# engcang/FAST-LIO-SAM-QN

Measured on AMD Instinct MI355X. Metric: scan-pair registrations/sec on 100k-pt clouds, higher is better.
Workload: dtype f32 search / f64 accumulate

## Files before the change

### fast-lio-sam-qn_amd/csrc/qn_context.h

```cpp
#pragma once
#include <hip/hip_runtime.h>
#include <string>
#include <vector>
#include "qn_gicp_kernels.cuh"

struct CloudBuf {
  uint32_t n = 0, ncells = 0;
  bool has_grid = false, has_cov = false;
  float4* raw = nullptr;
  float4* sorted = nullptr;
  float4* sorted_tmp = nullptr;
  uint32_t* cell_of_pt = nullptr;
  uint32_t* cell_start = nullptr;
  uint32_t* counts = nullptr;
  double* nrm = nullptr;
  qn::GridView grid{};
  qn::GridDims* dims = nullptr;
  qn::GridDims* dims_host = nullptr;
  const int32_t* knn_tab = nullptr; int knn_k = 0;
};

struct ProfSpan { int family; hipEvent_t a, b; int count; };

struct qn_ctx {
  int device = 0;
  uint32_t max_points = 0, max_cells = 0;
  hipStream_t stream = nullptr; bool owns_stream = true;
  std::vector<qn_ctx*> lanes; int batch_lanes = 8; char* args_h = nullptr; char* args_d = nullptr; size_t args_cap = 0; uint64_t batch_launches = 0, batch_pairs = 0; bool is_lane = false, batch_trace = false, batch_share_source = true;
  bool lanes_failed = false; int fail_lane_create = 0;
  void* slab = nullptr;
  qn_gicp_params params{};
  CloudBuf cloud[2];
  qn::BBoxAcc* bbox_acc = nullptr; qn::BBoxAcc* bbox_acc2 = nullptr;
  unsigned long long* scan_status = nullptr; unsigned long long* scan_status2 = nullptr; uint32_t build_epoch = 0;
  int far_group = -1;
  int far_chunk = 2;
  bool batch_look = false;
  bool far_ranked = true;
  unsigned long long* list_probe = nullptr;
  bool device_look = true;
  bool clear_far_now = false;
  char* staging2 = nullptr;
  struct PinZone { char* h = nullptr; hipEvent_t ev = nullptr; bool busy = false; } pin_up, pin_up2;
  char* staging = nullptr;
  uint32_t* scan_sums = nullptr;

  qn::GicpState* state = nullptr;
  uint32_t gen = 0; int part_rows = 0;
  double* partials = nullptr;
  uint32_t* tail_ticket = nullptr;
  double* fit_psum = nullptr; uint32_t* fit_pcnt = nullptr;
  qn_iter_trace* trace = nullptr; uint32_t trace_len = 0;
  int32_t* corr = nullptr; int32_t* nn_idx = nullptr; int32_t* knn_idx = nullptr; float4* nn_ref = nullptr; double* nrm_s_sorted = nullptr; qn::TargetRec* tgt_rec = nullptr; float* sqd = nullptr; float* sqd_fit = nullptr;
  int32_t* far_cand = nullptr; float4* far_cand_ref = nullptr; float2* far_cand_b = nullptr; unsigned long long* far_req = nullptr; uint32_t* far_stats = nullptr; double* far_rows = nullptr; int far_mode = 2; bool far_enabled = true;
  uint2* fb_list = nullptr; uint2* big_list = nullptr; uint32_t* fb_count2 = nullptr;
  float4* aligned = nullptr; bool aligned_valid = false;
  double* pose_tmp = nullptr; float* guess_tmp = nullptr;
  qn::ResultBlock* result_host = nullptr; double* scalar_host = nullptr;
  int32_t* dbg_knn_idx = nullptr; float* dbg_knn_d2 = nullptr;
  qn_quatro_params qparams{}; bool qparams_set = false, q_ready = false; double q_last_scale = 1.0;
  float4* q_normals[2] = {nullptr, nullptr}; float* q_spfh[2] = {nullptr, nullptr}; float* q_fpfh_s[2] = {nullptr, nullptr}; float* q_fpfh[2] = {nullptr, nullptr};
  unsigned long long* q_key[2] = {nullptr, nullptr};
  float* q_pair[2] = {nullptr, nullptr}; uint32_t* q_pair_hash[2] = {nullptr, nullptr};
  uint32_t* q_hit = nullptr; uint32_t* q_list = nullptr; uint32_t* q_sel = nullptr; uint2* q_pairs = nullptr; uint32_t* q_counts = nullptr; double* q_T = nullptr;
  void* q_mm_c = nullptr; void* q_mm_q = nullptr; float* q_mm_qn = nullptr; uint32_t* q_mm_L = nullptr; unsigned long long* q_mm_table = nullptr; unsigned long long* q_mm_table_q = nullptr; bool feat_query_dedupe = false;
  uint32_t q_mm_mask = 0;
  uint2* q_mm_pairs = nullptr; uint32_t* q_mm_cnt = nullptr; uint32_t q_mm_cap = 0, q_mm_ncnt = 0; bool feat_mfma = true, feat_mm_retry = false; int feat_sample = 4 ; bool feat_verify = false; int feat_min_blocks = 1536; double q_wall_ms[3] = {0, 0, 0}; unsigned long long* q_mm_vkeys = nullptr; uint32_t* q_mm_vcnt = nullptr; uint32_t feat_fallbacks = 0, feat_survivors = 0;
  bool c2f_overlap = false;
  bool c2f_lanes_fpfh = false;
  bool tgt_early = true;
  bool quatro_fused = true;
  int normals_fg = 0, fpfh_fg = 0;
  float4* c2f_src = nullptr; float4* c2f_dst = nullptr;
  float* q_mean = nullptr; double* q_mean_psum = nullptr; void* q_host = nullptr;
  double cell_override = 0.0;
  int list_small = 6000;
  float big_ratio = 2.5f;
  bool fused_ticks = true;
  int nn_rounds = 1;
  int nn_lane = -1;
  int track_from_tick = 3;
  int fused_from_tick = 3;
  int unseeded_until = 3; bool count_far_now = false; int last_extra_unseeded = 0;
  int unseeded_cap = 10;
  int single_from_tick = 2;
  bool fused_final = true;
  int knn_rounds = 2;
  int knn_mm = 1;
  int knn_trips = 3;
  int knn_hist = 1;
  int big_blocks0 = 4096, fb_blocks0 = 512;
  float margin_nn_t0 = 0.f;
  float margin_nn = 1.f, margin_knn = 0.f;
  int margin_nn_cap = 3, margin_knn_cap = 5, ticks_per_chunk = 8; bool knn_single_all = false, stable_cells = true; int bbox_blocks = 64;
  hipStream_t stream2 = nullptr; hipEvent_t ev_pair = nullptr; bool pair_pipeline = true, pair_failed = false, tgt_on_stream2 = false, tgt_pending = false, no_pipe = false;
// ... 24 lines not shown
```

### fast-lio-sam-qn_amd/csrc/qn_device.cuh

```cuda
#pragma once
#include <hip/hip_runtime.h>
#include <stdint.h>

namespace qn {

#define QN_TX 8
#define QN_TY 4
#define QN_TZ 4
#define QN_TILE_CELLS 128

struct GridDims {
  float ox, oy, oz, cell, inv_cell, eps;
  int nx, ny, nz, ntx, nty, ntz;
  uint32_t n;
  uint32_t ncells, nonfinite, pad;
};
struct GridView {
  const float4* pts;
  const uint32_t* cell_start;
  uint32_t* dbg;
  float ox, oy, oz, cell, inv_cell, eps;
  int nx, ny, nz;
  int ntx, nty, ntz;
  uint32_t n;
  const GridDims* dims;
};
__device__ __forceinline__ int uni(int v) { return __builtin_amdgcn_readfirstlane(v); }
__device__ __forceinline__ uint32_t uni(uint32_t v) { return (uint32_t)__builtin_amdgcn_readfirstlane((int)v); }
__device__ __forceinline__ float uni(float v) { return __int_as_float(__builtin_amdgcn_readfirstlane(__float_as_int(v))); }
__device__ __forceinline__ double uni(double v) { union { double d; int i[2]; } u; u.d = v; u.i[0] = __builtin_amdgcn_readfirstlane(u.i[0]); u.i[1] = __builtin_amdgcn_readfirstlane(u.i[1]); return u.d; }
__device__ __forceinline__ GridView grid_resolve(GridView g) {
  const GridDims d = *g.dims;
  g.ox = uni(d.ox); g.oy = uni(d.oy); g.oz = uni(d.oz); g.cell = uni(d.cell); g.inv_cell = uni(d.inv_cell); g.eps = uni(d.eps);
  g.nx = uni(d.nx); g.ny = uni(d.ny); g.nz = uni(d.nz); g.ntx = uni(d.ntx); g.nty = uni(d.nty); g.ntz = uni(d.ntz); g.n = uni(d.n);
  return g;
}

template <class A> struct alignas(16) LaneEntry { A a; uint32_t nbx; uint32_t pad_[3]; };
template <class F>
__global__ void __launch_bounds__(F::TB, F::OCC) k_lanes(const LaneEntry<typename F::Args>* __restrict__ tab) {
  const LaneEntry<typename F::Args>* e = tab + blockIdx.y;
  const uint32_t nbx = e->nbx;
  if (blockIdx.x >= nbx) return;
  F::run(e->a, blockIdx.x, nbx);
}

#define QN_INF_KEY 0xFFFFFFFFFFFFFFFFull

__device__ __forceinline__ int clampi(int v, int lo, int hi) { return v < lo ? lo : (v > hi ? hi : v); }
__device__ __forceinline__ int cell_coord(float v, float o, float inv, int n) {
  return clampi((int)floorf((v - o) * inv), 0, n - 1);
}
__device__ __forceinline__ uint32_t cell_key(const GridView& g, int x, int y, int z) {
  const uint32_t tile = ((uint32_t)(z >> 2) * g.nty + (y >> 2)) * g.ntx + (x >> 3);
  return (tile << 7) | ((z & 3) << 5) | ((y & 3) << 3) | (x & 7);
}
__device__ __forceinline__ unsigned long long pack_key(float d2, uint32_t idx) {
  return ((unsigned long long)__float_as_uint(d2) << 32) | idx;
}
__device__ __forceinline__ float key_d2(unsigned long long k) { return __uint_as_float((uint32_t)(k >> 32)); }
__device__ __forceinline__ uint32_t key_idx(unsigned long long k) { return (uint32_t)k; }

typedef float qn_f2 __attribute__((ext_vector_type(2)));
__device__ __forceinline__ float sqdist(float qx, float qy, float qz, float px, float py, float pz) {
  const qn_f2 q = {qx, qy}, p = {px, py};
  const qn_f2 d = q - p;
  const qn_f2 d2 = d * d;
  const float dz = qz - pz;
  return (d2.x + d2.y) + dz * dz;
}

__device__ __forceinline__ int rfl(int v) { return __builtin_amdgcn_readfirstlane(v); }
__device__ __forceinline__ uint32_t rflu(uint32_t v) { return (uint32_t)__builtin_amdgcn_readfirstlane((int)v); }
__device__ __forceinline__ int rdlane(int v, int l) { return __builtin_amdgcn_readlane(v, l); }
__device__ __forceinline__ uint32_t rdlane(uint32_t v, int l) { return (uint32_t)__builtin_amdgcn_readlane((int)v, l); }
__device__ __forceinline__ float rdlane(float v, int l) { return __int_as_float(__builtin_amdgcn_readlane(__float_as_int(v), l)); }

#if defined(QN_INST_GROUP) && QN_INST_GROUP == 10
__device__ __forceinline__ int wave_min_i(int v) {
#pragma unroll
  for (int o = 32; o > 0; o >>= 1) { int t = __shfl_xor(v, o); v = t < v ? t : v; }
  return v;
}
__device__ __forceinline__ int wave_max_i(int v) {
#pragma unroll
  for (int o = 32; o > 0; o >>= 1) { int t = __shfl_xor(v, o); v = t > v ? t : v; }
  return v;
}
__device__ __forceinline__ unsigned long long wave_min_u64(unsigned long long v) {
#pragma unroll
  for (int o = 32; o > 0; o >>= 1) { unsigned long long t = __shfl_xor(v, o); v = t < v ? t : v; }
  return v;
}
__device__ __forceinline__ float wave_min_f(float v) {
#pragma unroll
  for (int o = 32; o > 0; o >>= 1) v = fminf(v, __shfl_xor(v, o));
  return v;
}
__device__ __forceinline__ float wave_max_f(float v) {
#pragma unroll
  for (int o = 32; o > 0; o >>= 1) v = fmaxf(v, __shfl_xor(v, o));
  return v;
}
#else
#define QN_DPP_LADDER(STEP) STEP(0x111, 0xF) STEP(0x112, 0xF) STEP(0x114, 0xF) STEP(0x118, 0xF) STEP(0x142, 0xA) STEP(0x143, 0xC)
__device__ __forceinline__ int wave_min_i(int v) {
#define QN_S(ctrl, rm) { const int t = __builtin_amdgcn_update_dpp(0x7fffffff, v, ctrl, rm, 0xF, false); v = t < v ? t : v; }
  QN_DPP_LADDER(QN_S)
// ... 777 lines not shown
```

### fast-lio-sam-qn_amd/csrc/qn_engine.hip

```cpp
#include <hip/hip_runtime.h>
#include <cfloat>
#include <cmath>
#include <cstdio>
#include <cstring>
#include <string>
#include <vector>
#include <atomic>
#include <thread>
#include <chrono>
#include "qn_instances.h"
#include "qn_context.h"
#include "qn_selftest.cuh"
#include "qn_pool.h"

using namespace qn;

#define HIPCHK(ctx, call)                                                                 \
  do { hipError_t e_ = (call);                                                            \
       if (e_ != hipSuccess) { (ctx)->set_error(#call, e_, __LINE__); return QN_ERR_HIP; } \
  } while (0)

void qn_ctx::set_error(const char* what, hipError_t e, int line) {
  char buf[512]; snprintf(buf, sizeof(buf), "%s -> %s (qn_engine.hip:%d)", what, hipGetErrorString(e), line);
  last_error = buf;
}

void qn_ctx::prof_begin(int family, int count) {
  if (!prof_on) return;
  if (prof_open) { prof_depth++; return; }
  ProfSpan sp; sp.family = family; sp.count = count;
  if (hipEventCreate(&sp.a) != hipSuccess) return;
  if (hipEventCreate(&sp.b) != hipSuccess) { hipEventDestroy(sp.a); return; }
  hipEventRecord(sp.a, stream);
  spans.push_back(sp);
  prof_open = true; prof_depth = 0;
}
void qn_ctx::prof_end() {
  if (!prof_on || spans.empty() || !prof_open) return;
  if (prof_depth > 0) { prof_depth--; return; }
  prof_open = false;
  hipEventRecord(spans.back().b, stream);
}
void qn_ctx::prof_collect() {
  for (auto& sp : spans) {
    float ms = 0; if (hipEventSynchronize(sp.b) == hipSuccess && hipEventElapsedTime(&ms, sp.a, sp.b) == hipSuccess) { stats[sp.family].total_ms += ms; stats[sp.family].launches += sp.count; }
    hipEventDestroy(sp.a); hipEventDestroy(sp.b);
  }
  spans.clear(); prof_open = false; prof_depth = 0;
}
struct ProfScope { qn_ctx* c; ProfScope(qn_ctx* c_, int fam) : c(c_) { c->prof_begin(fam); } ~ProfScope() { c->prof_end(); } };

extern "C" const char* qn_status_str(int s) {
  switch (s) {
    case QN_OK: return "ok"; case QN_ERR_INVALID_ARG: return "invalid argument"; case QN_ERR_EMPTY_CLOUD: return "empty cloud";
    case QN_ERR_CAPACITY: return "cloud exceeds context capacity"; case QN_ERR_NOT_READY: return "clouds/covariances not set";
    case QN_ERR_HIP: return "HIP runtime error"; case QN_ERR_NO_DEVICE: return "no gfx950 device (no CPU fallback)";
  }
  return "unknown status";
}
extern "C" const char* qn_last_error(const qn_ctx* ctx) { return ctx ? ctx->last_error.c_str() : "null context"; }

extern "C" void qn_gicp_default_params(qn_gicp_params* p) {
  if (!p) return;
  memset(p, 0, sizeof(*p));
  p->k_correspondences = 20; p->max_iterations = 64; p->max_corr_dist = (double)FLT_MAX;
  p->transformation_epsilon = 5e-4; p->rotation_epsilon = 2e-3; p->optimizer = QN_OPT_LM;
  p->lm_max_iterations = 10; p->lm_init_lambda_factor = 1e-9; p->force_iterations = 0;
  p->ransac_iterations = 0; p->ransac_outlier_threshold = 0.05; p->euclidean_fitness_epsilon = -DBL_MAX;
}

struct Slab {
  char* base = nullptr; size_t off = 0, cap = 0;
  template <class T> void take(T*& p, size_t bytes) {
    const size_t a = (off + 255) & ~(size_t)255;
    if (base) p = (T*)(base + a);
    off = a + bytes;
  }
};
static void carve_cloud(qn_ctx* c, Slab& sl, CloudBuf& b) {
  sl.take(b.raw, sizeof(float4) * c->max_points);
  sl.take(b.sorted, sizeof(float4) * c->max_points);
  sl.take(b.sorted_tmp, sizeof(float4) * c->max_points);
  sl.take(b.cell_of_pt, sizeof(uint32_t) * c->max_points);
  sl.take(b.cell_start, sizeof(uint32_t) * ((size_t)c->max_cells + 1));
  sl.take(b.counts, sizeof(uint32_t) * ((size_t)c->max_cells + 1));
  sl.take(b.nrm, sizeof(double) * 3 * c->max_points);
  sl.take(b.dims, sizeof(GridDims));
}

static int ctx_create(int device, uint32_t max_points, hipStream_t shared_stream, qn_ctx** out);
extern "C" int qn_ctx_create(int device, uint32_t max_points, qn_ctx** out) { return ctx_create(device, max_points, nullptr, out); }
static int ctx_create(int device, uint32_t max_points, hipStream_t shared_stream, qn_ctx** out) {
  if (!out || max_points == 0) return QN_ERR_INVALID_ARG;
  *out = nullptr;
  if (max_points > QN_CTX_MAX_POINTS) return QN_ERR_CAPACITY;
  int ndev = 0;
  if (hipGetDeviceCount(&ndev) != hipSuccess || ndev <= 0 || device < 0 || device >= ndev) return QN_ERR_NO_DEVICE;
  qn_ctx* c = new qn_ctx();
  c->device = device; c->max_points = max_points;
  size_t mc = (size_t)max_points * 16; if (mc < (1u << 18)) mc = 1u << 18; if (mc > (1u << 23)) mc = 1u << 23;
  c->max_cells = (uint32_t)mc;
  qn_gicp_default_params(&c->params);
  int rc = QN_OK;
  auto fail = [&](int code) { qn_ctx_destroy(c); return code; };
  if (hipSetDevice(device) != hipSuccess) return fail(QN_ERR_NO_DEVICE);
  if (shared_stream) { c->stream = shared_stream; c->owns_stream = false; c->is_lane = true; }
  else if (hipStreamCreateWithFlags(&c->stream, hipStreamNonBlocking) != hipSuccess) return fail(QN_ERR_HIP);
#define CA(call) if ((call) != hipSuccess) return fail(QN_ERR_HIP)
  auto carve = [&](Slab& sl) {
    carve_cloud(c, sl, c->cloud[0]);
    carve_cloud(c, sl, c->cloud[1]);
    sl.take(c->staging, (size_t)max_points * 32);
    sl.take(c->scan_sums, sizeof(uint32_t) * (c->max_cells / (QN_BLOCK * QN_SCAN_ITEMS) + 2));
    sl.take(c->state, 2 * sizeof(GicpState));
    sl.take(c->partials, 2 * sizeof(double) * (QN_ACC_MAX_BLOCKS + 8) * QN_NPART);
    sl.take(c->nn_idx, sizeof(int32_t) * max_points);
    sl.take(c->knn_idx, sizeof(int32_t) * (size_t)max_points * 32);
    sl.take(c->nn_ref, sizeof(float4) * max_points);
    sl.take(c->nrm_s_sorted, sizeof(double) * 3 * max_points);
    sl.take(c->tgt_rec, sizeof(TargetRec) * max_points);
    sl.take(c->fit_psum, sizeof(double) * (QN_ACC_MAX_BLOCKS + 8));
    sl.take(c->fit_pcnt, sizeof(uint32_t) * (QN_ACC_MAX_BLOCKS + 8));
    sl.take(c->trace, sizeof(qn_iter_trace) * QN_MAX_TRACE);
    sl.take(c->corr, sizeof(int32_t) * max_points);
    sl.take(c->sqd, sizeof(float) * max_points);
    sl.take(c->sqd_fit, sizeof(float) * max_points);
    sl.take(c->far_cand, sizeof(int32_t) * QN_FAR_M * (size_t)max_points);
    sl.take(c->far_cand_ref, sizeof(float4) * max_points);
    sl.take(c->far_cand_b, sizeof(float2) * max_points);
    sl.take(c->far_req, sizeof(unsigned long long) * (max_points / 64 + 2));
    sl.take(c->far_stats, 4 * sizeof(uint32_t));
    sl.take(c->far_rows, sizeof(double) * QN_FAR_BLOCKS * QN_NPART);
    sl.take(c->fb_list, sizeof(uint2) * max_points);
    sl.take(c->big_list, sizeof(uint2) * max_points);
    sl.take(c->fb_count2, 4 * sizeof(uint32_t));
    sl.take(c->aligned, sizeof(float4) * max_points);
    sl.take(c->pose_tmp, sizeof(double) * 16);
    sl.take(c->guess_tmp, sizeof(float) * 16);
    sl.take(c->scan_sums2, sizeof(uint32_t) * (c->max_cells / (QN_BLOCK * QN_SCAN_ITEMS) + 2));
    sl.take(c->fb_list2, sizeof(uint2) * max_points);
    sl.take(c->big_list2, sizeof(uint2) * max_points);
    sl.take(c->fb_count2b, 4 * sizeof(uint32_t));
    sl.take(c->knn_idx2, sizeof(int32_t) * (size_t)max_points * 32);
    sl.take(c->staging2, (size_t)max_points * 32);
    sl.take(c->bbox_acc, 2 * (QN_BBOX_MAX_BLOCKS + 1) * sizeof(BBoxAcc)); c->bbox_acc2 = c->bbox_acc ? c->bbox_acc + (QN_BBOX_MAX_BLOCKS + 1) : nullptr;
    sl.take(c->scan_status, sizeof(unsigned long long) * 2 * (c->max_cells / (QN_BLOCK * QN_SCAN_ITEMS) + 2)); c->scan_status2 = c->scan_status ? c->scan_status + (c->max_cells / (QN_BLOCK * QN_SCAN_ITEMS) + 2) : nullptr;
    sl.take(c->pg_rows, sizeof(unsigned long long) * 3 * QN_PERSIST_ROWS * QN_PERSIST_RSTRIDE);
    sl.take(c->pg_bc, sizeof(unsigned long long) * 64);
    sl.take(c->pg_fit, sizeof(unsigned long long) * (QN_PERSIST_MAX_BLOCKS + 1) * 4);
    sl.take(c->pg_status, 4 * sizeof(uint32_t));
    sl.take(c->tail_ticket, 4 * sizeof(uint32_t));
  };
  { Slab dry; carve(dry);
    Slab sl; sl.cap = (dry.off + ((size_t)2 << 20) - 1) & ~(((size_t)2 << 20) - 1);
    CA(hipMalloc(&c->slab, sl.cap)); sl.base = (char*)c->slab; carve(sl); }
  CA(hipMemsetAsync(c->far_stats, 0, 4 * sizeof(uint32_t), c->stream));
  CA(hipHostMalloc(&c->result_host, sizeof(ResultBlock), hipHostMallocDefault));
  for (int w = 0; w < 2; w++) { CA(hipHostMalloc(&c->cloud[w].dims_host, sizeof(GridDims), hipHostMallocDefault)); memset(c->cloud[w].dims_host, 0, sizeof(GridDims)); }
  CA(hipHostMalloc(&c->scalar_host, 64 * sizeof(double), hipHostMallocDefault));
  CA(hipHostMalloc(&c->pg_status_host, 4 * sizeof(uint32_t), hipHostMallocDefault));
  CA(hipMemsetAsync(c->pg_rows, 0xFF, sizeof(unsigned long long) * 3 * QN_PERSIST_ROWS * QN_PERSIST_RSTRIDE, c->stream));
  CA(hipMemsetAsync(c->pg_bc, 0, sizeof(unsigned long long) * 64, c->stream));
  CA(hipMemsetAsync(c->pg_fit, 0, sizeof(unsigned long long) * (QN_PERSIST_MAX_BLOCKS + 1) * 4, c->stream));
  CA(hipMemsetAsync(c->pg_status, 0, 4 * sizeof(uint32_t), c->stream));
  CA(hipMemsetAsync(c->tail_ticket, 0, 4 * sizeof(uint32_t), c->stream));
  CA(hipMemsetAsync(c->state, 0, 2 * sizeof(GicpState), c->stream));
// ... 29 lines not shown
  hipFree(c->q_mm_c); hipFree(c->q_mm_q); hipFree(c->q_mm_qn); hipFree(c->q_mm_L); hipFree(c->q_mm_table); hipFree(c->q_mm_table_q); hipFree(c->q_mm_pairs); hipFree(c->q_mm_cnt); hipFree(c->q_mm_vkeys); hipFree(c->q_mm_vcnt);
  for (int w = 0; w < 2; w++) { hipFree(c->q_normals[w]); hipFree(c->q_spfh[w]); hipFree(c->q_fpfh_s[w]); hipFree(c->q_fpfh[w]); hipFree(c->q_key[w]); hipFree(c->q_pair[w]); hipFree(c->q_pair_hash[w]); }
  hipFree(c->q_hit); hipFree(c->q_list); hipFree(c->q_sel); hipFree(c->q_pairs); hipFree(c->q_counts); hipFree(c->q_T); hipFree(c->q_mean); hipFree(c->q_mean_psum);
  if (c->q_host) hipHostFree(c->q_host);
  hipFree(c->c2f_src); hipFree(c->c2f_dst);
  hipFree(c->dbg_knn_idx); hipFree(c->dbg_knn_d2); hipFree(c->dbg_counters);
  hipFree(c->v_corr); hipFree(c->v_nn_idx); hipFree(c->v_sqd); hipFree(c->v_nn_ref); hipFree(c->v_counters);
  if (c->result_host) hipHostFree(c->result_host);
  for (int w = 0; w < 2; w++) if (c->cloud[w].dims_host) hipHostFree(c->cloud[w].dims_host);
  if (c->scalar_host) hipHostFree(c->scalar_host);
  hipFree(c->pg_clk); if (c->list_probe) hipFree(c->list_probe); if (c->pg_status_host) hipHostFree(c->pg_status_host);
  if (c->ev_pair) hipEventDestroy(c->ev_pair);
  for (qn_ctx::PinZone* z : {&c->pin_up, &c->pin_up2}) { if (z->ev) hipEventDestroy(z->ev); if (z->h) hipHostFree(z->h); }
  if (c->stream2) { hipStreamSynchronize(c->stream2); hipStreamDestroy(c->stream2); }
  if (c->stream && c->owns_stream) hipStreamDestroy(c->stream);
  delete c;
}

static int clouds_valid(qn_ctx* c);
extern "C" void* qn_ctx_stream(qn_ctx* c) { return c ? (void*)c->stream : nullptr; }
int qn_ctx_int_device(const qn_ctx* c) { return c->device; }
extern "C" int qn_ctx_synchronize(qn_ctx* c) {
  if (!c) return QN_ERR_INVALID_ARG;
  HIPCHK(c, hipStreamSynchronize(c->stream));
  if (c->stream2) HIPCHK(c, hipStreamSynchronize(c->stream2));
  c->prof_collect();
  return clouds_valid(c);
}

extern "C" int qn_gicp_set_params(qn_ctx* c, const qn_gicp_params* p) {
  if (!c || !p) return QN_ERR_INVALID_ARG;
  if (p->k_correspondences < 1 || p->k_correspondences > 32 || p->max_iterations < 0 || p->lm_max_iterations < 1 ||
      (p->optimizer != QN_OPT_LM && p->optimizer != QN_OPT_GN) || !(p->max_corr_dist > 0) || !(p->lm_init_lambda_factor >= 0)) return QN_ERR_INVALID_ARG;
  if (p->k_correspondences != c->params.k_correspondences) { c->cloud[0].has_cov = c->cloud[1].has_cov = false; }
  c->params = *p;
  return QN_OK;
}

extern "C" int qn_gicp_get_params(const qn_ctx* c, qn_gicp_params* p) { if (!c || !p) return QN_ERR_INVALID_ARG; *p = c->params; return QN_OK; }

static GicpConfig make_cfg(const qn_ctx* c) {
  GicpConfig g; const qn_gicp_params& p = c->params;
  g.k = p.k_correspondences; g.max_iterations = p.max_iterations; g.optimizer = p.optimizer; g.lm_max_iterations = p.lm_max_iterations;
  g.force_iterations = p.force_iterations; g.max_corr_dist_sq = p.max_corr_dist * p.max_corr_dist;
  g.transformation_epsilon = p.transformation_epsilon; g.rotation_epsilon = p.rotation_epsilon; g.lm_init_lambda_factor = p.lm_init_lambda_factor;
  return g;
}

static inline GicpState* st_cur(qn_ctx* c) { return c->state + (c->gen & 1u); }
static inline GicpState* st_nxt(qn_ctx* c) { return c->state + ((c->gen + 1u) & 1u); }
static inline double* part_cur(qn_ctx* c) { return c->partials + (size_t)(c->gen & 1u) * (QN_ACC_MAX_BLOCKS + 8) * QN_NPART; }
static inline double* part_nxt(qn_ctx* c) { return c->partials + (size_t)((c->gen + 1u) & 1u) * (QN_ACC_MAX_BLOCKS + 8) * QN_NPART; }

static bool pair_pipeline_ready(qn_ctx* c) {
  if (c->stream2) return true;
  if (c->pair_failed || !c->knn_idx2) return false;
  const bool ok = hipStreamCreateWithFlags(&c->stream2, hipStreamNonBlocking) == hipSuccess && hipEventCreateWithFlags(&c->ev_pair, hipEventDisableTiming) == hipSuccess;
  if (!ok) { c->pair_failed = true; if (c->stream2) { hipStreamDestroy(c->stream2); c->stream2 = nullptr; } (void)hipGetLastError(); }
  return ok;
}
static void swap_scratch(qn_ctx* c) {
  std::swap(c->stream, c->stream2); std::swap(c->scan_sums, c->scan_sums2); std::swap(c->fb_list, c->fb_list2); std::swap(c->big_list, c->big_list2);
  std::swap(c->fb_count2, c->fb_count2b); std::swap(c->knn_idx, c->knn_idx2);
  std::swap(c->bbox_acc, c->bbox_acc2); std::swap(c->scan_status, c->scan_status2);
  std::swap(c->pin_up, c->pin_up2);
  std::swap(c->staging, c->staging2);
}
struct TargetScope {
  qn_ctx* c; bool on;
  TargetScope(qn_ctx* c_, bool on_) : c(c_), on(on_) { if (on) swap_scratch(c); }
  ~TargetScope() { if (on) { (void)hipEventRecord(c->ev_pair, c->stream); swap_scratch(c); c->tgt_pending = true; } }
};
static int join_target(qn_ctx* c) {
  if (!c->tgt_pending) return QN_OK;
  c->tgt_pending = false;
  return hipStreamWaitEvent(c->stream, c->ev_pair, 0) == hipSuccess ? QN_OK : QN_ERR_HIP;
}

struct GridLaunch { PackBBoxK::Args pack; uint32_t pack_nb; CellCountK::Args count; ScanLookbackK::Args scan; uint32_t scan_nb; ScatterK::Args scat; StableCellsK::Args stab; bool stable; uint32_t nb; };
static GridLaunch prep_grid(qn_ctx* c, CloudBuf& b, const char* dsrc, uint32_t stride, bool lanes = false) {
  const uint32_t n = b.n;
  GridView& g = b.grid;
  memset(&g, 0, sizeof(g));
  g.pts = b.sorted; g.cell_start = b.cell_start; g.dbg = c->dbg_counters; g.n = n; g.dims = b.dims;
  GridLaunch L;
  L.nb = (n + QN_BLOCK - 1) / QN_BLOCK;
  L.scan_nb = (c->max_cells + QN_BLOCK * QN_SCAN_ITEMS - 1) / (QN_BLOCK * QN_SCAN_ITEMS);
  if (((++c->build_epoch) & 0x3fffffffu) == 0u) ++c->build_epoch;
  L.pack_nb = std::min<uint32_t>(L.nb, (uint32_t)std::min(lanes ? QN_BBOX_MAX_BLOCKS : c->bbox_blocks, QN_BBOX_MAX_BLOCKS));
  L.pack = PackBBoxK::Args{dsrc, stride, n, b.raw, c->bbox_acc, c->max_cells, c->cell_override, b.dims, b.dims_host};
  L.count = CellCountK::Args{b.raw, n, g, b.counts, b.cell_of_pt};
  L.scan = ScanLookbackK::Args{b.counts, b.dims, b.cell_start, c->scan_status, c->build_epoch, n};
  L.stable = c->stable_cells;
  L.scat = ScatterK::Args{b.raw, n, b.cell_of_pt, b.cell_start, b.counts, L.stable ? b.sorted_tmp : b.sorted};
  L.stab = StableCellsK::Args{b.sorted_tmp, n, b.cell_of_pt, b.cell_start, b.sorted};
  b.has_grid = true; b.has_cov = false; b.knn_tab = nullptr;
  return L;
}
static int build_grid(qn_ctx* c, CloudBuf& b, const char* dsrc, uint32_t stride) {
  hipStream_t s = c->stream;
  const GridLaunch L = prep_grid(c, b, dsrc, stride);
  { ProfScope ps(c, QN_K_GRID_BUILD);
    hipLaunchKernelGGL(k_pack_bbox_dims, dim3(L.pack_nb), dim3(QN_BLOCK), 0, s, L.pack.in, L.pack.stride, L.pack.n, L.pack.raw, L.pack.acc, L.pack.max_cells, L.pack.cell_override, L.pack.dims_dev, L.pack.dims_host);
    hipLaunchKernelGGL(k_cell_count, dim3(L.nb), dim3(QN_BLOCK), 0, s, L.count.pts, L.count.n, L.count.g, L.count.counts, L.count.cell_of_pt);
    hipLaunchKernelGGL(k_scan_lookback, dim3(L.scan_nb), dim3(QN_BLOCK), 0, s, L.scan.in, L.scan.dims, L.scan.out, L.scan.status, L.scan.epoch, L.scan.total);
    hipLaunchKernelGGL(k_scatter, dim3(L.nb), dim3(QN_BLOCK), 0, s, L.scat.pts, L.scat.n, L.scat.cell_of_pt, L.scat.cell_start, L.scat.counts, L.scat.sorted);
    if (L.stable) hipLaunchKernelGGL(k_stable_cells, dim3(L.nb), dim3(QN_BLOCK), 0, s, L.stab.in, L.stab.n, L.stab.cell_of_pt, L.stab.cell_start, L.stab.out); }
  HIPCHK(c, hipGetLastError());
  return QN_OK;
}
static int clouds_valid(qn_ctx* c) {
  for (int w = 0; w < 2; w++)
    if (c->cloud[w].has_grid && c->cloud[w].dims_host && c->cloud[w].dims_host->nonfinite) {
      c->last_error = w == 0 ? "source cloud contains non-finite coordinates (is_dense == false clouds are not supported)" : "target cloud contains non-finite coordinates (is_dense == false clouds are not supported)";
      c->cloud[w].has_grid = c->cloud[w].has_cov = false;
      return QN_ERR_INVALID_ARG;
    }
  return QN_OK;
}

static int upload_host_cloud(qn_ctx* c, const float* xyz, uint32_t n, uint32_t& stride, hipStream_t s, const char** dsrc) {
  hipPointerAttribute_t at;
  const bool pinned = hipPointerGetAttributes(&at, xyz) == hipSuccess && at.type == hipMemoryTypeHost;
  if (!pinned) (void)hipGetLastError();
  if (pinned) {
    if (stride <= 32) { HIPCHK(c, hipMemcpyAsync(c->staging, xyz, (size_t)(n - 1) * stride + 12, hipMemcpyHostToDevice, s)); }
    else { HIPCHK(c, hipMemcpy2DAsync(c->staging, 16, xyz, stride, 16, n, hipMemcpyHostToDevice, s)); stride = 16; }
    *dsrc = (const char*)c->staging;
    return QN_OK;
  }
  qn_ctx::PinZone& z = c->pin_up;
  if (!z.h) { HIPCHK(c, hipHostMalloc((void**)&z.h, (size_t)c->max_points * 16, hipHostMallocDefault)); HIPCHK(c, hipEventCreateWithFlags(&z.ev, hipEventDisableTiming)); }
  if (z.busy) { HIPCHK(c, hipEventSynchronize(z.ev)); z.busy = false; }
  float* o = (float*)z.h; const char* in = (const char*)xyz;
  for (uint32_t i = 0; i < n; i++, in += stride, o += 3) { const float* p = (const float*)in; o[0] = p[0]; o[1] = p[1]; o[2] = p[2]; }
  HIPCHK(c, hipMemcpyAsync(c->staging, z.h, (size_t)n * 12, hipMemcpyHostToDevice, s));
  HIPCHK(c, hipEventRecord(z.ev, s)); z.busy = true;
  stride = 12; *dsrc = (const char*)c->staging;
  return QN_OK;
}

static int set_cloud(qn_ctx* c, int which, const float* xyz, uint32_t n, uint32_t stride, bool on_device) {
  if (!c || (which != 0 && which != 1)) return QN_ERR_INVALID_ARG;
  CloudBuf& b = c->cloud[which];
  b.n = 0; b.has_grid = b.has_cov = false;
  if (n == 0) return QN_ERR_EMPTY_CLOUD;
  if (!xyz || stride < 12 || (stride & 3)) return QN_ERR_INVALID_ARG;
  if (n > c->max_points) return QN_ERR_CAPACITY;
  HIPCHK(c, hipSetDevice(c->device));
  if (which == QN_SOURCE && join_target(c) != QN_OK) return QN_ERR_HIP;
  c->tgt_on_stream2 = which == QN_TARGET ? (c->pair_pipeline && !c->prof_on && !c->no_pipe && c->cloud[0].has_grid && pair_pipeline_ready(c)) : c->tgt_on_stream2;
  TargetScope scope(c, which == QN_TARGET && c->tgt_on_stream2);
  hipStream_t s = c->stream;
  const char* dsrc = (const char*)xyz;
  if (!on_device) { const int rc = upload_host_cloud(c, xyz, n, stride, s, &dsrc); if (rc != QN_OK) return rc; }
  b.n = n;
  return build_grid(c, b, dsrc, stride);
}

extern "C" int qn_gicp_set_source(qn_ctx* c, const float* xyz, uint32_t n, uint32_t stride) { return set_cloud(c, QN_SOURCE, xyz, n, stride, false); }
extern "C" int qn_gicp_set_target(qn_ctx* c, const float* xyz, uint32_t n, uint32_t stride) { return set_cloud(c, QN_TARGET, xyz, n, stride, false); }
extern "C" int qn_gicp_set_source_device(qn_ctx* c, const float* xyz, uint32_t n, uint32_t stride) { return set_cloud(c, QN_SOURCE, xyz, n, stride, true); }
extern "C" int qn_gicp_set_target_device(qn_ctx* c, const float* xyz, uint32_t n, uint32_t stride) { return set_cloud(c, QN_TARGET, xyz, n, stride, true); }

struct KnnLaunch { KnnHistArgs sel; uint32_t sel_nb; KnnHistArgs lst; uint32_t lst_nb; KnnSingleK::Args single; uint32_t single_nb; KnnCovArgs tail; uint32_t tail_nb; CovFromIdxK::Args cov; uint32_t cov_nb; };
static float knn_first_radius(const qn_ctx* c, const CloudBuf& b) {
  return -(c->margin_knn > 0.f ? c->margin_knn : (b.n > 16384u && b.n <= 65536u ? 2.5f : 2.0f));
}
static KnnLaunch prep_knn(qn_ctx* c, CloudBuf& b, int k, int32_t* kidx, float* kd2, bool lanes = false) {
  const float r0 = knn_first_radius(c, b);
  uint32_t* genc = c->fb_count2 + 1;
  KnnLaunch L;
  L.sel_nb = (b.n + QN_KNN_BLOCK / 4 - 1) / (QN_KNN_BLOCK / 4);
  if (lanes && c->knn_trips > 1) L.sel_nb = (L.sel_nb + (uint32_t)c->knn_trips - 1) / (uint32_t)c->knn_trips;
  L.sel = KnnHistArgs{b.grid, k, r0, c->knn_single_all ? -1 : c->knn_rounds, kidx, kd2, c->fb_list, c->fb_count2, c->big_list, genc};
  L.lst_nb = std::min<uint32_t>((b.n + 63) / 64, lanes ? 96 : 512) * (QN_BLOCK / QN_KNN_BLOCK);
  L.lst = KnnHistArgs{b.grid, k, r0, 64, kidx, kd2, c->fb_list, c->fb_count2, c->big_list, genc};
  L.single_nb = std::min<uint32_t>((b.n + 3) / 4, lanes ? 128 : 2048);
  L.single = KnnSingleK::Args{b.grid, k, kidx, kd2, c->big_list, genc, c->fb_list, c->fb_count2 + 2};
  L.tail_nb = std::min<uint32_t>((b.n + 63) / 64, lanes ? 64 : 1024);
  L.tail = KnnCovArgs{b.grid, b.raw, k, r0, 64, b.nrm, kidx, kd2, c->fb_list, c->fb_count2 + 2};
  L.cov_nb = (b.n + QN_BLOCK - 1) / QN_BLOCK;
  L.cov = CovFromIdxK::Args{b.raw, b.sorted, b.n, k, kidx, b.nrm, &b == &c->cloud[0] ? c->nrm_s_sorted : (double*)nullptr, &b == &c->cloud[0] ? (TargetRec*)nullptr : c->tgt_rec, c->fb_count2};
  return L;
}
template <int KMAX>
static void launch_knn_cov(qn_ctx* c, CloudBuf& b, int k, int32_t* kidx, float* kd2) {
  hipStream_t s = c->stream;
  if (c->knn_hist) {
    const KnnLaunch L = prep_knn(c, b, k, kidx, kd2);
    constexpr int HCAP = KMAX <= 24 ? 32 : 48;
    { ProfScope sel(c, QN_K_KNN_SELECT);
      if (!c->knn_mm) hipLaunchKernelGGL(HIP_KERNEL_NAME(k_knn_hist<false, HCAP, false>), dim3(L.sel_nb), dim3(QN_KNN_BLOCK), 0, s, L.sel.g, L.sel.k, L.sel.r0, L.sel.max_rounds, L.sel.knn_idx, L.sel.knn_d2, L.sel.fb_list, L.sel.fb_count, L.sel.gen_list, L.sel.gen_count);
      else hipLaunchKernelGGL(HIP_KERNEL_NAME(k_knn_hist<false, HCAP>), dim3(L.sel_nb), dim3(QN_KNN_BLOCK), 0, s, L.sel.g, L.sel.k, L.sel.r0, L.sel.max_rounds, L.sel.knn_idx, L.sel.knn_d2, L.sel.fb_list, L.sel.fb_count, L.sel.gen_list, L.sel.gen_count); }
    ProfScope ps(c, QN_K_KNN_COV);
    if (!c->knn_mm) hipLaunchKernelGGL(HIP_KERNEL_NAME(k_knn_hist<true, HCAP, false>), dim3(L.lst_nb), dim3(QN_KNN_BLOCK), 0, s, L.lst.g, L.lst.k, L.lst.r0, L.lst.max_rounds, L.lst.knn_idx, L.lst.knn_d2, L.lst.fb_list, L.lst.fb_count, L.lst.gen_list, L.lst.gen_count);
    else hipLaunchKernelGGL(HIP_KERNEL_NAME(k_knn_hist<true, HCAP>), dim3(L.lst_nb), dim3(QN_KNN_BLOCK), 0, s, L.lst.g, L.lst.k, L.lst.r0, L.lst.max_rounds, L.lst.knn_idx, L.lst.knn_d2, L.lst.fb_list, L.lst.fb_count, L.lst.gen_list, L.lst.gen_count);
    hipLaunchKernelGGL(k_knn_single, dim3(L.single_nb), dim3(QN_BLOCK), 0, s, L.single.g, L.single.k, L.single.knn_idx, L.single.knn_d2, L.single.list, L.single.count, L.single.gen_list, L.single.gen_count);
    hipLaunchKernelGGL(HIP_KERNEL_NAME(k_knn_cov<KMAX, true, 4>), dim3(L.tail_nb), dim3(QN_BLOCK), 0, s, L.tail.g, L.tail.raw, L.tail.k, L.tail.r0, L.tail.max_rounds, L.tail.cov, L.tail.knn_idx, L.tail.knn_d2, L.tail.fb_list, L.tail.fb_count);
    hipLaunchKernelGGL(k_cov_from_idx, dim3(L.cov_nb), dim3(QN_BLOCK), 0, s, L.cov.raw, L.cov.sorted, L.cov.n, L.cov.k, L.cov.knn_idx, L.cov.nrm, L.cov.nrm_sorted, L.cov.rec, L.cov.list_counts);
    return;
  }
  const float r0 = knn_first_radius(c, b);
  ProfScope ps(c, QN_K_KNN_COV);
  {
    const uint32_t nb = (b.n + QN_BLOCK / 4 - 1) / (QN_BLOCK / 4);
    hipLaunchKernelGGL(HIP_KERNEL_NAME(k_knn_cov<KMAX, false, 4>), dim3(nb), dim3(QN_BLOCK), 0, s, b.grid, b.raw, k, r0, 2, b.nrm, kidx, kd2, c->fb_list, c->fb_count2);
  }
  hipLaunchKernelGGL(HIP_KERNEL_NAME(k_knn_cov<KMAX, true, 4>), dim3(std::min<uint32_t>((b.n + 63) / 64, 512)), dim3(QN_BLOCK), 0, s, b.grid, b.raw, k, r0, 64, b.nrm, kidx, kd2, c->fb_list, c->fb_count2);
  const uint32_t nbp = (b.n + QN_BLOCK - 1) / QN_BLOCK;
  hipLaunchKernelGGL(k_cov_from_idx, dim3(nbp), dim3(QN_BLOCK), 0, s, b.raw, b.sorted, b.n, k, kidx, b.nrm,
                     &b == &c->cloud[0] ? c->nrm_s_sorted : (double*)nullptr, &b == &c->cloud[0] ? (TargetRec*)nullptr : c->tgt_rec, c->fb_count2);
}
static void note_knn_table(qn_ctx* c, CloudBuf& b, const int32_t* kidx, int k) {
  for (CloudBuf& o : c->cloud) if (&o != &b && o.knn_tab == kidx) o.knn_tab = nullptr;
  b.knn_tab = kidx; b.knn_k = k;
}
static int compute_cov(qn_ctx* c, int which, int32_t* kidx, float* kd2) {
  if (!c || (which != 0 && which != 1)) return QN_ERR_INVALID_ARG;
  CloudBuf& b = c->cloud[which];
  if (!b.has_grid) return b.n == 0 ? QN_ERR_EMPTY_CLOUD : QN_ERR_NOT_READY;
  HIPCHK(c, hipSetDevice(c->device));
  const int k = c->params.k_correspondences;
  const bool on2 = which == QN_TARGET && c->tgt_on_stream2 && !c->prof_on && kidx == c->knn_idx && c->stream2 != nullptr;
  if (which == QN_TARGET && !on2 && join_target(c) != QN_OK) return QN_ERR_HIP;
  if (on2) kidx = c->knn_idx2;
  TargetScope scope(c, on2);
  if (k <= 16) launch_knn_cov<16>(c, b, k, kidx, kd2);
  else if (k <= 20) launch_knn_cov<20>(c, b, k, kidx, kd2);
  else if (k <= 24) launch_knn_cov<24>(c, b, k, kidx, kd2);
  else launch_knn_cov<32>(c, b, k, kidx, kd2);
  HIPCHK(c, hipGetLastError());
  b.has_cov = true;
  if (kidx == c->knn_idx || kidx == c->knn_idx2) note_knn_table(c, b, kidx, k);
  return QN_OK;
}
extern "C" int qn_gicp_compute_covariances(qn_ctx* c, int which) { return compute_cov(c, which, c->knn_idx, nullptr); }

struct NnLaunch { NnSearchArgs grid; uint32_t grid_nb; NnSearchArgs list; uint32_t list_nb; bool group; bool lane; };
static NnLaunch prep_nn(qn_ctx* c, int mode , float* sqd_out, bool seeded, int tick, int cond) {
  CloudBuf &S = c->cloud[0], &T = c->cloud[1];
  const uint32_t nb = (S.n + QN_NN_BLOCK / 4 - 1) / (QN_NN_BLOCK / 4);
  const uint32_t nb4 = (S.n + QN_BLOCK / 4 - 1) / (QN_BLOCK / 4);
  const double thr2 = c->params.max_corr_dist * c->params.max_corr_dist;
  GicpState* st = st_cur(c);
  uint32_t* fbc = &st->fb_count; uint32_t* bgc = &st->big_count;
  uint32_t* far_stats = (mode == 0 && !seeded && c->count_far_now) ? c->far_stats : nullptr;
  const bool wide = tick <= 2 || (mode == 0 && !seeded);
  int big_blocks = wide ? c->big_blocks0 : 1024;
  const uint32_t fbb = std::min<uint32_t>(nb4, wide ? (uint32_t)c->fb_blocks0 : 256u);
  const float r0 = -(tick == 0 && mode == 0 && c->margin_nn_t0 > 0.f ? c->margin_nn_t0 : c->margin_nn);
  const float big_ratio = c->big_ratio;
  NnOpt opt; opt.clear_ref = (mode == 0 && !seeded && c->clear_far_now) ? c->far_cand_ref : nullptr; opt.cond = cond;
  const bool batch = c->persist_batch_off;
  opt.group = c->far_group >= 0 ? c->far_group : (batch ? 2048 : 0); opt.group_min = 0;
  if (mode == 0 && opt.group > 0) big_blocks = std::min(big_blocks, std::max(64, (opt.group + QN_BLOCK / 64 - 1) / (QN_BLOCK / 64)));
  opt.probe = (mode == 0 && !seeded) ? c->list_probe : nullptr;
  opt.fb_small = (mode == 0 && !c->persist_batch_off) ? (uint32_t)c->list_small : 0u;
  NnOpt opt0; opt0.clear_ref = nullptr; opt0.cond = 0; opt0.group = 0; opt0.group_min = 0; opt0.probe = nullptr; opt0.fb_small = 0;
  c->clear_far_now = mode == 0 && !seeded ? false : c->clear_far_now;
  const NnOpt& o = mode == 0 ? opt : opt0;
  NnLaunch L;
  L.lane = (c->nn_lane > 0 || (c->nn_lane < 0 && c->persist_batch_off)) && mode == 0 && !seeded;
  L.grid_nb = L.lane ? (S.n + 255u) / 256u : nb; L.list_nb = fbb + (uint32_t)big_blocks; L.group = mode == 0 && opt.group > 0;
  L.grid = NnSearchArgs{S.grid, T.grid, st, thr2, r0, mode == 0 ? c->nn_rounds : 1, c->corr, sqd_out, c->nn_idx, c->nn_ref, c->fb_list, fbc, c->big_list, bgc, 0, big_ratio, far_stats, o};
  L.list = NnSearchArgs{S.grid, T.grid, st, thr2, r0, 64, c->corr, sqd_out, c->nn_idx, c->nn_ref, c->fb_list, fbc, c->big_list, bgc, big_blocks, big_ratio, far_stats, o};
  return L;
}
#define QN_NN_ARGS(A) A.src, A.tgt, A.st, A.thr2, A.r0, A.max_rounds, A.corr, A.sqd, A.nn_idx, A.nn_ref, A.fb_list, A.fb_count, A.big_list, A.big_count, A.big_blocks, A.big_ratio, A.far_stats, A.opt
static void enqueue_nn(qn_ctx* c, int mode , float* sqd_out, bool seeded, int tick = 0, int cond = 0) {
  hipStream_t s = c->stream;
  CloudBuf &S = c->cloud[0], &T = c->cloud[1];
  const uint32_t nbt = (S.n + QN_BLOCK - 1) / QN_BLOCK;
  const NnLaunch L = prep_nn(c, mode, sqd_out, seeded, tick, cond);
  if (L.grid.opt.probe) (void)hipMemsetAsync(c->list_probe, 0, sizeof(unsigned long long) * 4 * 16384, s);
  const NnSearchArgs& G = L.grid; const NnSearchArgs& F = L.list;
  if (mode == 0) {
    { ProfScope ps(c, QN_K_NN_SEARCH);
      if (seeded) hipLaunchKernelGGL(HIP_KERNEL_NAME(k_nn_track<0>), dim3(nbt), dim3(QN_BLOCK), 0, s, S.grid, T.grid, T.raw, G.st, G.thr2, c->corr, sqd_out, c->nn_idx, c->nn_ref, c->fb_list, G.fb_count, c->big_list, G.big_count);
      else if (L.lane) hipLaunchKernelGGL(HIP_KERNEL_NAME(k_nn_lane<0>), dim3(L.grid_nb), dim3(256), 0, s, G);
      else hipLaunchKernelGGL(HIP_KERNEL_NAME(k_nn_search<0, false, QN_NN_BLOCK>), dim3(L.grid_nb), dim3(QN_NN_BLOCK), 0, s, QN_NN_ARGS(G)); }
    { ProfScope ps(c, QN_K_NN_FALLBACK);
      if (L.group) hipLaunchKernelGGL(HIP_KERNEL_NAME(k_nn_search<0, true, QN_BLOCK, true>), dim3(L.list_nb), dim3(QN_BLOCK), 0, s, QN_NN_ARGS(F));
      else hipLaunchKernelGGL(HIP_KERNEL_NAME(k_nn_search<0, true, QN_BLOCK>), dim3(L.list_nb), dim3(QN_BLOCK), 0, s, QN_NN_ARGS(F)); }
  } else {
    ProfScope ps(c, QN_K_FITNESS);
    if (seeded) hipLaunchKernelGGL(HIP_KERNEL_NAME(k_nn_track<1>), dim3(nbt), dim3(QN_BLOCK), 0, s, S.grid, T.grid, T.raw, G.st, G.thr2, c->corr, sqd_out, c->nn_idx, c->nn_ref, c->fb_list, G.fb_count, c->big_list, G.big_count);
    else hipLaunchKernelGGL(HIP_KERNEL_NAME(k_nn_search<1, false, QN_NN_BLOCK>), dim3(L.grid_nb), dim3(QN_NN_BLOCK), 0, s, QN_NN_ARGS(G));
    hipLaunchKernelGGL(HIP_KERNEL_NAME(k_nn_search<1, true, QN_BLOCK>), dim3(L.list_nb), dim3(QN_BLOCK), 0, s, QN_NN_ARGS(F));
  }
}
static void enqueue_verify(qn_ctx* c, bool fused) {
  hipStream_t s = c->stream;
  CloudBuf &S = c->cloud[0], &T = c->cloud[1];
// ... 405 lines not shown
                                      qn_gicp_result* results, int* valid, int* status) {
  if (!ctxs || n_ctx == 0 || (n_pairs && (!pairs || !results || !valid || !status))) return QN_ERR_INVALID_ARG;
  for (uint32_t i = 0; i < n_ctx; i++) if (!ctxs[i]) return QN_ERR_INVALID_ARG;
  std::atomic<uint32_t> next{0}, final_share{0};
  std::vector<char> saved(n_ctx);
  std::vector<char> saved_p(n_ctx);
  std::vector<char> use_lanes(n_ctx);
  for (uint32_t i = 0; i < n_ctx; i++) {
    saved[i] = ctxs[i]->pair_pipeline; saved_p[i] = ctxs[i]->persist_batch_off;
    use_lanes[i] = n_pairs > 1 && batch_supported(ctxs[i]) && batch_ensure_lanes(ctxs[i]) == QN_OK;
    if (n_ctx > 1 || use_lanes[i]) { ctxs[i]->pair_pipeline = false; ctxs[i]->persist_batch_off = true; }
  }
  auto worker = [&](qn_ctx* c, bool lanes) {
    if (lanes) {
      (void)hipSetDevice(c->device);
      (void)join_target(c);
      const uint32_t B = (uint32_t)c->lanes.size();
      std::vector<const float*> last_src(B, nullptr); std::vector<uint64_t> last_key(B, 0);
      std::vector<uint32_t> idx(B);
      for (;;) {
        uint32_t base = next.load(), m = 0;
        for (;;) {
          if (base >= n_pairs) break;
          const uint32_t rem = n_pairs - base;
          if (rem > n_ctx * B) m = B;
          else {
            uint32_t q = final_share.load();
            if (q == 0) { uint32_t want = std::min<uint32_t>(B, std::max<uint32_t>((uint32_t)std::max(1, ctxs[0]->batch_min_share), (rem + n_ctx - 1) / n_ctx)); if (final_share.compare_exchange_strong(q, want)) q = want; }
            m = std::min(q, rem);
          }
          m = std::min(m, B);
          if (next.compare_exchange_weak(base, base + m)) break;
        }
        if (base >= n_pairs) break;
        for (uint32_t l = 0; l < m; l++) idx[l] = base + l;
        const int rc = batch_register(c, pairs, idx.data(), m, thr, results, valid, status, last_src, last_key, nullptr);
        if (rc != QN_OK) { (void)hipStreamSynchronize(c->stream); for (uint32_t l = 0; l < m; l++) status[base + l] = rc; std::fill(last_src.begin(), last_src.end(), nullptr); }
      }
      return;
    }
    const qn_pair_desc* last = nullptr;
    for (;;) {
      const uint32_t i = next.fetch_add(1);
      if (i >= n_pairs) break;
      const qn_pair_desc& p = pairs[i];
      const bool same = c->batch_share_source && last && last->src == p.src && last->ns == p.ns && last->stride_bytes == p.stride_bytes && last->on_device == p.on_device;
      status[i] = icp_alignment(c, p.src, p.ns, p.dst, p.nt, p.stride_bytes, thr, &results[i], &valid[i], p.on_device ? 1 : 0, same);
      last = status[i] == QN_OK ? &p : nullptr;
    }
  };
  qn::WorkerPool::instance().run(n_ctx, [&](uint32_t i) { worker(ctxs[i], use_lanes[i] != 0); });
  for (uint32_t i = 0; i < n_ctx; i++) { ctxs[i]->pair_pipeline = saved[i] != 0; ctxs[i]->persist_batch_off = saved_p[i] != 0; }
  return QN_OK;
}

extern "C" int qn_gicp_get_covariances(qn_ctx* c, int which, double* out9) {
  if (c && join_target(c) != QN_OK) return QN_ERR_HIP;
  if (!c || !out9 || (which != 0 && which != 1)) return QN_ERR_INVALID_ARG;
  CloudBuf& b = c->cloud[which];
  if (!b.has_cov) return QN_ERR_NOT_READY;
  HIPCHK(c, hipSetDevice(c->device));
  std::vector<double> h((size_t)b.n * 6);
  double* d6 = nullptr;
  HIPCHK(c, hipMalloc(&d6, sizeof(double) * 6 * b.n));
  hipLaunchKernelGGL(k_cov_from_normals, dim3((b.n + 255) / 256), dim3(256), 0, c->stream, b.nrm, b.n, d6);
  hipError_t ce = hipMemcpyAsync(h.data(), d6, sizeof(double) * 6 * b.n, hipMemcpyDeviceToHost, c->stream);
  if (ce == hipSuccess) ce = hipStreamSynchronize(c->stream);
  (void)hipFree(d6);
  if (ce != hipSuccess) { c->set_error("covariance read-back", ce, __LINE__); return QN_ERR_HIP; }
  { const int vrc = clouds_valid(c); if (vrc != QN_OK) return vrc; }
  for (uint32_t i = 0; i < b.n; i++) {
    const double* s = &h[(size_t)i * 6]; double* o = out9 + (size_t)i * 9;
    o[0] = s[0]; o[1] = s[1]; o[2] = s[2]; o[3] = s[1]; o[4] = s[3]; o[5] = s[4]; o[6] = s[2]; o[7] = s[4]; o[8] = s[5];
  }
  return QN_OK;
}

static int lane_ctx(qn_ctx* c, uint32_t lane, qn_ctx** out) {
  if (c->lanes.empty()) { if (lane != 0) return QN_ERR_NOT_READY; *out = c; return QN_OK; }
  if (lane >= c->lanes.size()) return QN_ERR_INVALID_ARG;
  *out = c->lanes[lane];
  return QN_OK;
}
extern "C" int qn_gicp_get_lane_knn(qn_ctx* c, uint32_t lane, int which, int32_t* idx_out, uint32_t* n, int* k) {
  if (c && join_target(c) != QN_OK) return QN_ERR_HIP;
  if (!c || !n || !k || (which != 0 && which != 1)) return QN_ERR_INVALID_ARG;
  *n = 0; *k = 0;
  qn_ctx* l = nullptr;
  { const int rc = lane_ctx(c, lane, &l); if (rc != QN_OK) return rc; }
  const CloudBuf& b = l->cloud[which];
  if (!b.has_grid || !b.has_cov || !b.knn_tab || b.knn_k != c->params.k_correspondences) return QN_ERR_NOT_READY;
  *n = b.n; *k = b.knn_k;
  if (!idx_out) return QN_OK;
  HIPCHK(c, hipSetDevice(c->device));
  HIPCHK(c, hipMemcpyAsync(idx_out, b.knn_tab, sizeof(int32_t) * (size_t)b.n * b.knn_k, hipMemcpyDeviceToHost, l->stream));
  HIPCHK(c, hipStreamSynchronize(l->stream));
  return clouds_valid(l);
}
extern "C" int qn_gicp_get_lane_covariances(qn_ctx* c, uint32_t lane, int which, double* cov9_out) {
  if (!c) return QN_ERR_INVALID_ARG;
  qn_ctx* l = nullptr;
  { const int rc = lane_ctx(c, lane, &l); if (rc != QN_OK) return rc; }
  if (l != c && join_target(c) != QN_OK) return QN_ERR_HIP;
  return qn_gicp_get_covariances(l, which, cov9_out);
}

extern "C" int qn_gicp_knn(qn_ctx* c, int which, int k, int32_t* idx_out, float* d2_out) {
  if (c && join_target(c) != QN_OK) return QN_ERR_HIP;
  if (!c || !idx_out || !d2_out || (which != 0 && which != 1) || k < 1 || k > 32) return QN_ERR_INVALID_ARG;
  CloudBuf& b = c->cloud[which];
  if (!b.has_grid) return QN_ERR_NOT_READY;
  HIPCHK(c, hipSetDevice(c->device));
  hipFree(c->dbg_knn_idx); hipFree(c->dbg_knn_d2); c->dbg_knn_idx = nullptr; c->dbg_knn_d2 = nullptr;
  HIPCHK(c, hipMalloc(&c->dbg_knn_idx, sizeof(int32_t) * (size_t)b.n * k));
  HIPCHK(c, hipMalloc(&c->dbg_knn_d2, sizeof(float) * (size_t)b.n * k));
  HIPCHK(c, hipMemsetAsync(c->dbg_knn_idx, 0xff, sizeof(int32_t) * (size_t)b.n * k, c->stream));
  const int ksave = c->params.k_correspondences; const bool had = b.has_cov;
  c->params.k_correspondences = k;
  int rc = compute_cov(c, which, c->dbg_knn_idx, c->dbg_knn_d2);
  c->params.k_correspondences = ksave;
  b.has_cov = had && (k == ksave);
  if (rc != QN_OK) return rc;
  HIPCHK(c, hipMemcpyAsync(idx_out, c->dbg_knn_idx, sizeof(int32_t) * (size_t)b.n * k, hipMemcpyDeviceToHost, c->stream));
  HIPCHK(c, hipMemcpyAsync(d2_out, c->dbg_knn_d2, sizeof(float) * (size_t)b.n * k, hipMemcpyDeviceToHost, c->stream));
  HIPCHK(c, hipStreamSynchronize(c->stream));
  c->prof_collect();
  return clouds_valid(c);
}

extern "C" int qn_gicp_linearize(qn_ctx* c, const double T[16], double H[36], double b6[6], double* err, int32_t* corr_out, float* sqd_out) {
  if (c && join_target(c) != QN_OK) return QN_ERR_HIP;
  int rc = ready(c); if (rc != QN_OK) return rc;
  if (!T || !H || !b6 || !err) return QN_ERR_INVALID_ARG;
  HIPCHK(c, hipSetDevice(c->device));
  hipStream_t s = c->stream;
  HIPCHK(c, hipMemcpyAsync(c->pose_tmp, T, sizeof(double) * 16, hipMemcpyHostToDevice, s));
  hipLaunchKernelGGL(k_set_pose, dim3(1), dim3(64), 0, s, st_cur(c), c->pose_tmp, 0, 0);
  enqueue_nn(c, 0, c->sqd, false); enqueue_accumulate(c, 0, false); enqueue_solve(c, 1, 0);
  GicpState* hs = (GicpState*)malloc(sizeof(GicpState));
  hipError_t e = hipMemcpyAsync(hs, st_cur(c), sizeof(GicpState), hipMemcpyDeviceToHost, s);
  if (e == hipSuccess && corr_out) e = hipMemcpyAsync(corr_out, c->corr, sizeof(int32_t) * c->cloud[0].n, hipMemcpyDeviceToHost, s);
  if (e == hipSuccess && sqd_out) e = hipMemcpyAsync(sqd_out, c->sqd, sizeof(float) * c->cloud[0].n, hipMemcpyDeviceToHost, s);
  if (e == hipSuccess) e = hipStreamSynchronize(s);
  if (e != hipSuccess) { free(hs); c->set_error("linearize readback", e, __LINE__); return QN_ERR_HIP; }
  memcpy(H, hs->H, sizeof(double) * 36); memcpy(b6, hs->b, sizeof(double) * 6); *err = hs->y0;
  free(hs);
  c->prof_collect();
  return clouds_valid(c);
}

extern "C" int qn_gicp_compute_error(qn_ctx* c, const double T[16], double* err) {
  if (c && join_target(c) != QN_OK) return QN_ERR_HIP;
  int rc = ready(c); if (rc != QN_OK) return rc;
  if (!T || !err) return QN_ERR_INVALID_ARG;
  HIPCHK(c, hipSetDevice(c->device));
  hipStream_t s = c->stream;
  HIPCHK(c, hipMemcpyAsync(c->pose_tmp, T, sizeof(double) * 16, hipMemcpyHostToDevice, s));
  hipLaunchKernelGGL(k_set_pose, dim3(1), dim3(64), 0, s, st_cur(c), c->pose_tmp, 1, 1);
  enqueue_accumulate(c, 0, false); enqueue_solve(c, 2, 0);
  HIPCHK(c, hipMemcpyAsync(c->scalar_host, &st_cur(c)->yi, sizeof(double), hipMemcpyDeviceToHost, s));
  HIPCHK(c, hipStreamSynchronize(s));
  *err = c->scalar_host[0];
  c->prof_collect();
  return clouds_valid(c);
}

extern "C" int qn_prof_enable(qn_ctx* c, int on) { if (!c) return QN_ERR_INVALID_ARG; c->prof_on = on != 0; return QN_OK; }
extern "C" int qn_prof_reset(qn_ctx* c) { if (!c) return QN_ERR_INVALID_ARG; c->prof_collect(); for (auto& s : c->stats) { s.total_ms = 0; s.launches = 0; } return QN_OK; }
extern "C" int qn_prof_get(qn_ctx* c, int fam, qn_kernel_stat* out) {
  if (!c || !out || fam < 0 || fam >= QN_K_COUNT) return QN_ERR_INVALID_ARG;
  c->prof_collect(); *out = c->stats[fam]; return QN_OK;
}
extern "C" int qn_debug_set(qn_ctx* c, const char* key, double v) {
  if (!c || !key) return QN_ERR_INVALID_ARG;
  std::string k(key);
  if (k == "cell") { c->cell_override = v; c->cloud[0].has_grid = c->cloud[1].has_grid = false; }
  else if (k == "margin_nn") c->margin_nn = (float)v;
  else if (k == "margin_nn_t0") c->margin_nn_t0 = (float)v;
  else if (k == "big_blocks0") c->big_blocks0 = v < 64 ? 64 : (int)v;
  else if (k == "fb_blocks0") c->fb_blocks0 = v < 64 ? 64 : (int)v;
  else if (k == "margin_knn") c->margin_knn = (float)v;
  else if (k == "knn_single_all") c->knn_single_all = v != 0;
  else if (k == "bbox_blocks") c->bbox_blocks = std::max(1, (int)v);
  else if (k == "device_look") c->device_look = v != 0;
  else if (k == "far_group") c->far_group = (int)v;
  else if (k == "c2f_overlap") c->c2f_overlap = v != 0;
  else if (k == "quatro_fused") c->quatro_fused = v != 0;
  else if (k == "tgt_early") c->tgt_early = v != 0;
  else if (k == "c2f_lanes_fpfh") c->c2f_lanes_fpfh = v != 0;
  else if (k == "normals_fg") c->normals_fg = (int)v;
  else if (k == "fpfh_fg") c->fpfh_fg = (int)v;
  else if (k == "list_small") c->list_small = std::max(0, (int)v);
  else if (k == "far_chunk") c->far_chunk = std::max(1, (int)v);
  else if (k == "far_ranked") c->far_ranked = v != 0;
  else if (k == "batch_look") c->batch_look = v != 0;
  else if (k == "unseeded_cap") c->unseeded_cap = (int)v;
  else if (k == "pair_pipeline") c->pair_pipeline = v != 0;
  else if (k == "persist") c->persist = v != 0;
  else if (k == "persist_timeout") c->persist_timeout = v < 1 ? 1ull : (unsigned long long)v;
  else if (k == "prof_persist") c->prof_persist = v != 0;
  else if (k == "persist_probe") {
    if (v != 0 && !c->pg_clk) { if (hipMalloc(&c->pg_clk, 8 * (64 * 16 + 16)) != hipSuccess) return QN_ERR_HIP; }
    if (c->pg_clk) (void)hipMemset(c->pg_clk, 0, 8 * (64 * 16 + 16));
    if (v == 0) { (void)hipFree(c->pg_clk); c->pg_clk = nullptr; }
  }
  else if (k == "batch_lanes") {
    const int b = std::max(1, std::min((int)v, 64));
    if (b < (int)c->lanes.size()) { if (hipStreamSynchronize(c->stream) != hipSuccess) return QN_ERR_HIP; while ((int)c->lanes.size() > std::max(b, 1)) { qn_ctx* l = c->lanes.back(); c->lanes.pop_back(); if (l != c) qn_ctx_destroy(l); } }
// ... 61 lines not shown
}
extern "C" int qn_debug_selftest(qn_ctx* c, uint32_t n_waves, uint32_t seed, uint32_t* mismatches) {
  if (!c || !mismatches || n_waves == 0 || n_waves > 65536) return QN_ERR_INVALID_ARG;
  HIPCHK(c, hipSetDevice(c->device));
  std::vector<uint32_t> h((size_t)n_waves * 128);
  uint64_t x = 0x9e3779b97f4a7c15ull ^ seed;
  for (auto& v : h) { x ^= x << 13; x ^= x >> 7; x ^= x << 17; v = (uint32_t)(x >> 16); }
  uint32_t* d = nullptr;
  HIPCHK(c, hipMalloc(&d, (h.size() + 1) * sizeof(uint32_t)));
  int rc = QN_OK; uint32_t bad = 0xffffffffu;
  if (hipMemcpyAsync(d, h.data(), h.size() * sizeof(uint32_t), hipMemcpyHostToDevice, c->stream) != hipSuccess || hipMemsetAsync(d + h.size(), 0, sizeof(uint32_t), c->stream) != hipSuccess) rc = QN_ERR_HIP;
  if (rc == QN_OK) {
    hipLaunchKernelGGL(k_selftest_wave, dim3(n_waves), dim3(64), 0, c->stream, d, d + (size_t)n_waves * 64, d + h.size());
    if (hipMemcpyAsync(&bad, d + h.size(), sizeof(uint32_t), hipMemcpyDeviceToHost, c->stream) != hipSuccess || hipStreamSynchronize(c->stream) != hipSuccess) rc = QN_ERR_HIP;
  }
  (void)hipFree(d);
  if (rc != QN_OK) { c->last_error = "selftest: HIP call failed"; return rc; }
  *mismatches = bad;
  return QN_OK;
}
extern "C" int qn_debug_get_counters(qn_ctx* c, uint32_t out[16]) {
  if (!c || !c->dbg_counters) return QN_ERR_INVALID_ARG;
  if (hipStreamSynchronize(c->stream) != hipSuccess) return QN_ERR_HIP;
  if (hipMemcpy(out, c->dbg_counters, 16 * sizeof(uint32_t), hipMemcpyDeviceToHost) != hipSuccess) return QN_ERR_HIP;
  return QN_OK;
}
extern "C" int qn_debug_get(qn_ctx* c, const char* key, double* value) {
  if (!c || !key || !value) return QN_ERR_INVALID_ARG;
  const std::string k(key);
  if (k == "verify_mismatches" || k == "verify_passes" || k == "verify_first") {
    if (!c->v_counters) return QN_ERR_NOT_READY;
    uint32_t h[4];
    if (hipStreamSynchronize(c->stream) != hipSuccess || hipMemcpy(h, c->v_counters, 16, hipMemcpyDeviceToHost) != hipSuccess) return QN_ERR_HIP;
    *value = k == "verify_mismatches" ? h[0] : (k == "verify_passes" ? h[1] : h[2]);
    return QN_OK;
  }
  if (k == "feat_mismatches" || k == "feat_verified" || k == "feat_first_mismatch") {
    if (!c->q_mm_vcnt) return QN_ERR_NOT_READY;
    uint32_t h[4];
    if (hipStreamSynchronize(c->stream) != hipSuccess || hipMemcpy(h, c->q_mm_vcnt, 16, hipMemcpyDeviceToHost) != hipSuccess) return QN_ERR_HIP;
    *value = k == "feat_mismatches" ? h[0] : (k == "feat_verified" ? h[2] : h[1]);
    return QN_OK;
  }
  if (k == "quatro_wall_features_ms") { *value = c->q_wall_ms[0]; return QN_OK; }
  if (k == "quatro_wall_match_ms") { *value = c->q_wall_ms[1]; return QN_OK; }
  if (k == "quatro_wall_solve_ms") { *value = c->q_wall_ms[2]; return QN_OK; }
  if (k == "extra_unseeded") { *value = c->last_extra_unseeded; return QN_OK; }
  if (k == "normals_width") { *value = c->quatro_normals_width(); return QN_OK; }
  if (k == "fpfh_width") { *value = c->quatro_fpfh_width(); return QN_OK; }
  if (k == "persist_launches") { *value = c->persist_launches; return QN_OK; }
  if (k == "persist_gave_up") { *value = c->persist_gave_up; return QN_OK; }
  if (k == "persist_fits") { *value = c->persist_fits ? 1 : 0; return QN_OK; }
  if (k == "persist_resident_blocks") { *value = c->persist_resident_blocks; return QN_OK; }
  if (k == "batch_launches") { *value = (double)c->batch_launches; return QN_OK; }
  if (k == "batch_pairs") { *value = (double)c->batch_pairs; return QN_OK; }
  if (k == "lanes_failed") { *value = c->lanes_failed ? 1.0 : 0.0; return QN_OK; }
  if (k == "batch_lanes") { *value = (double)c->batch_lanes; return QN_OK; }
  if (k == "feat_fallbacks") { *value = c->feat_fallbacks; return QN_OK; }
  if (k == "feat_survivors") { *value = c->feat_survivors; return QN_OK; }
  return QN_ERR_INVALID_ARG;
}
extern "C" int qn_debug_get_clk(qn_ctx* c, unsigned long long* out , uint32_t* n) {
  if (!c || !out || !n || !c->clk_probe) return QN_ERR_INVALID_ARG;
  if (hipStreamSynchronize(c->stream) != hipSuccess || hipMemcpy(out, c->clk_probe, 8 * 8 * 256 + 8 * 12 * 1024, hipMemcpyDeviceToHost) != hipSuccess) return QN_ERR_HIP;
  *n = c->clk_n; return QN_OK;
}
extern "C" int qn_debug_get_list_probe(qn_ctx* c, unsigned long long* out ) {
  if (!c || !out || !c->list_probe) return QN_ERR_INVALID_ARG;
  if (hipStreamSynchronize(c->stream) != hipSuccess || hipMemcpy(out, c->list_probe, sizeof(unsigned long long) * 4 * 16384, hipMemcpyDeviceToHost) != hipSuccess) return QN_ERR_HIP;
  return QN_OK;
}
extern "C" int qn_debug_get_persist_clk(qn_ctx* c, unsigned long long* out ) {
  if (!c || !out || !c->pg_clk) return QN_ERR_INVALID_ARG;
  if (hipStreamSynchronize(c->stream) != hipSuccess || hipMemcpy(out, c->pg_clk, 8 * (64 * 16 + 16), hipMemcpyDeviceToHost) != hipSuccess) return QN_ERR_HIP;
  return QN_OK;
}
extern "C" int qn_debug_get_partials(qn_ctx* c, double* out , uint32_t* rows_per_buffer, double* state ) {
  if (!c || !out || !rows_per_buffer || !state) return QN_ERR_INVALID_ARG;
  *rows_per_buffer = QN_ACC_MAX_BLOCKS + 8;
  if (hipStreamSynchronize(c->stream) != hipSuccess || hipMemcpy(out, c->partials, 2 * sizeof(double) * (QN_ACC_MAX_BLOCKS + 8) * QN_NPART, hipMemcpyDeviceToHost) != hipSuccess
      || hipMemcpy(state, c->state, 2 * sizeof(GicpState), hipMemcpyDeviceToHost) != hipSuccess) return QN_ERR_HIP;
  return QN_OK;
}
extern "C" int qn_debug_get_grid(qn_ctx* c, int which, double out[8]) {
  if (!c || (which != 0 && which != 1) || !c->cloud[which].has_grid) return QN_ERR_INVALID_ARG;
  if (hipStreamSynchronize(c->stream) != hipSuccess || (c->stream2 && hipStreamSynchronize(c->stream2) != hipSuccess)) return QN_ERR_HIP;
  const GridDims& g = *c->cloud[which].dims_host;
  out[0] = g.ox; out[1] = g.oy; out[2] = g.oz; out[3] = g.cell; out[4] = g.nx; out[5] = g.ny; out[6] = g.nz; out[7] = g.eps;
  return QN_OK;
}

#include "qn_batch.inc"
#include "qn_quatro_host.inc"
#include "qn_kf_quatro.inc"
#include "qn_kf_submap.inc"
```

### fast-lio-sam-qn_amd/csrc/qn_gicp_kernels.cuh

```cuda
#pragma once
#include "qn_device.cuh"
#include "qn_knn_hist.cuh"
#include "../../include/qn_engine.h"
#include "qn_util_kernels.cuh"

namespace qn {

#define QN_NPART 28
#define QN_ACC_MAX_BLOCKS 512
#define QN_MAX_TRACE 1024

struct GicpState {
  double x0[16], xi[16], delta[16];
  double H[36], b[6], d[6];
  double y0, yi, den;
  double lambda, nu;
  double final_H[36];
  double fitness;
  int outer, inner, phase, converged, lm_failed;
  uint32_t fb_count;
  uint32_t trace_len;
  uint32_t big_count;
  int pending;
  int reserved;
// ... 120 lines not shown
}

#define QN_LB_STATE_AGG 1ull
#define QN_LB_STATE_INC 2ull
struct ScanLookbackK {
  static constexpr int TB = QN_BLOCK, OCC = 1;
  struct Args { const uint32_t* in; const GridDims* dims; uint32_t* out; unsigned long long* status; uint32_t epoch, total; };
  static __device__ __forceinline__ void run(const Args& a, const uint32_t bx, const uint32_t) {
    __shared__ uint32_t wsum[QN_BLOCK / 64];
    __shared__ uint32_t s_prefix;
    const uint32_t* __restrict__ in = a.in; uint32_t* __restrict__ out = a.out; unsigned long long* status = a.status;
    const uint32_t total = a.total;
    const uint32_t m = uni(a.dims->ncells);
    const uint32_t tile = bx;
    if (tile * (uint32_t)(QN_BLOCK * QN_SCAN_ITEMS) >= m) return;
    const uint32_t base = (tile * QN_BLOCK + threadIdx.x) * QN_SCAN_ITEMS;
    uint32_t v[QN_SCAN_ITEMS], s = 0;
    if (base + QN_SCAN_ITEMS <= m) {
      const uint4* q = (const uint4*)(in + base);
#pragma unroll
      for (int j = 0; j < QN_SCAN_ITEMS / 4; j++) { const uint4 x = q[j]; v[4 * j] = x.x; v[4 * j + 1] = x.y; v[4 * j + 2] = x.z; v[4 * j + 3] = x.w; }
    } else {
#pragma unroll
      for (int j = 0; j < QN_SCAN_ITEMS; j++) v[j] = (base + j < m) ? in[base + j] : 0u;
    }
#pragma unroll
    for (int j = 0; j < QN_SCAN_ITEMS; j++) s += v[j];
    uint32_t inc = s;
    const int lane = threadIdx.x & 63, wid = threadIdx.x >> 6;
#pragma unroll
    for (int o = 1; o < 64; o <<= 1) { uint32_t t = __shfl_up(inc, o); if (lane >= o) inc += t; }
    if (lane == 63) wsum[wid] = inc;
    __syncthreads();
    uint32_t woff = 0, agg = 0;
    for (int w = 0; w < QN_BLOCK / 64; w++) { if (w < wid) woff += wsum[w]; agg += wsum[w]; }
    const unsigned long long tag = (unsigned long long)(a.epoch & 0x3fffffffu) << 34;
    if (wid == 0) {
      uint32_t prefix = 0;
      if (tile == 0) {
        if (lane == 0) __hip_atomic_store(status, tag | (QN_LB_STATE_INC << 32) | agg, __ATOMIC_RELAXED, __HIP_MEMORY_SCOPE_AGENT);
      } else {
        if (lane == 0) __hip_atomic_store(status + tile, tag | (QN_LB_STATE_AGG << 32) | agg, __ATOMIC_RELAXED, __HIP_MEMORY_SCOPE_AGENT);
        int look = (int)tile - 1;
        for (;;) {
          const int mine = look - lane;
          unsigned long long x = 0;
          if (mine >= 0) { do { x = __hip_atomic_load(status + mine, __ATOMIC_RELAXED, __HIP_MEMORY_SCOPE_AGENT); } while ((x >> 34) != (tag >> 34)); }
          const bool is_inc = mine >= 0 && ((x >> 32) & 3ull) == QN_LB_STATE_INC;
          const unsigned long long incs = __ballot(is_inc);
          const int first = incs ? __ffsll((long long)incs) - 1 : 64;
          uint32_t part = (mine >= 0 && lane <= first) ? (uint32_t)x : 0u;
#pragma unroll
          for (int o = 32; o > 0; o >>= 1) part += __shfl_xor(part, o);
          prefix += part;
          if (incs || look - 64 < 0) break;
          look -= 64;
        }
        if (lane == 0) __hip_atomic_store(status + tile, tag | (QN_LB_STATE_INC << 32) | (prefix + agg), __ATOMIC_RELAXED, __HIP_MEMORY_SCOPE_AGENT);
      }
      if (lane == 0) s_prefix = prefix;
    }
    __syncthreads();
    uint32_t run = s_prefix + woff + inc - s;
    if (base + QN_SCAN_ITEMS <= m) {
      uint4* q = (uint4*)(out + base);
#pragma unroll
      for (int j = 0; j < QN_SCAN_ITEMS / 4; j++) { uint4 x; x.x = run; run += v[4 * j]; x.y = run; run += v[4 * j + 1]; x.z = run; run += v[4 * j + 2]; x.w = run; run += v[4 * j + 3]; q[j] = x; }
    } else {
#pragma unroll
      for (int j = 0; j < QN_SCAN_ITEMS; j++) { if (base + j < m) out[base + j] = run; run += v[j]; }
    }
    if (base <= m && m < base + QN_SCAN_ITEMS) out[m] = total;
    if (m == (tile + 1u) * (uint32_t)(QN_BLOCK * QN_SCAN_ITEMS) && threadIdx.x == QN_BLOCK - 1) out[m] = total;
  }
};
static __global__ void __launch_bounds__(QN_BLOCK) k_scan_lookback(const uint32_t* __restrict__ in, const GridDims* __restrict__ dims, uint32_t* __restrict__ out,
                                                                   unsigned long long* status, uint32_t epoch, uint32_t total) {
  const ScanLookbackK::Args a{in, dims, out, status, epoch, total};
  ScanLookbackK::run(a, blockIdx.x, gridDim.x);
}

struct ScatterK {
  static constexpr int TB = QN_BLOCK, OCC = 1;
  struct Args { const float4* pts; uint32_t n; const uint32_t* cell_of_pt; const uint32_t* cell_start; uint32_t* counts; float4* sorted; };
  static __device__ __forceinline__ void run(const Args& a, const uint32_t bx, const uint32_t) {
    const uint32_t i = bx * QN_BLOCK + threadIdx.x;
    if (i >= a.n) return;
    const uint32_t c = a.cell_of_pt[i];
    const uint32_t slot = a.cell_start[c] + atomicSub(&a.counts[c], 1u) - 1u;
    float4 p = a.pts[i];
    p.w = __uint_as_float(i);
    a.sorted[slot] = p;
  }
};
static __global__ void __launch_bounds__(QN_BLOCK) k_scatter(const float4* __restrict__ pts, uint32_t n, const uint32_t* __restrict__ cell_of_pt,
                          const uint32_t* __restrict__ cell_start, uint32_t* __restrict__ counts, float4* __restrict__ sorted) {
  const ScatterK::Args a{pts, n, cell_of_pt, cell_start, counts, sorted};
  ScatterK::run(a, blockIdx.x, gridDim.x);
}

struct StableCellsK {
  static constexpr int TB = QN_BLOCK, OCC = 1;
  struct Args { const float4* in; uint32_t n; const uint32_t* cell_of_pt; const uint32_t* cell_start; float4* out; };
  static __device__ __forceinline__ void run(const Args& a, const uint32_t bx, const uint32_t) {
    const float4* __restrict__ in = a.in; float4* __restrict__ out = a.out;
    const uint32_t t = bx * QN_BLOCK + threadIdx.x;
    if (t >= a.n) return;
    const float4 p = in[t];
    const uint32_t i = __float_as_uint(p.w), c = a.cell_of_pt[i];
    const uint32_t s = a.cell_start[c], e = a.cell_start[c + 1];
    if (e - s > 256u) { out[t] = p; return; }
    uint32_t rank = 0;
    for (uint32_t u = s; u < e; u++) rank += __float_as_uint(in[u].w) < i ? 1u : 0u;
    out[s + rank] = p;
  }
};
static __global__ void __launch_bounds__(QN_BLOCK) k_stable_cells(const float4* __restrict__ in, uint32_t n, const uint32_t* __restrict__ cell_of_pt, const uint32_t* __restrict__ cell_start,
                                      float4* __restrict__ out) {
  const StableCellsK::Args a{in, n, cell_of_pt, cell_start, out};
  StableCellsK::run(a, blockIdx.x, gridDim.x);
}

struct __attribute__((aligned(64))) TargetRec { float4 p; double n[3]; double pad[3]; };
static_assert(sizeof(TargetRec) == 64, "TargetRec is one 64-byte line");
#define QN_COV_BATCH 10
#define QN_COV_REG 20
struct CovFromIdxK {
  static constexpr int TB = QN_BLOCK, OCC = 1;
  struct Args { const float4* raw; const float4* sorted; uint32_t n; int k; const int32_t* knn_idx; double* nrm; double* nrm_sorted; TargetRec* rec; uint32_t* list_counts; };
  static __device__ __forceinline__ void run(const Args& a, const uint32_t bx, const uint32_t nbx) {
    const float4* __restrict__ raw = a.raw; const int32_t* __restrict__ knn_idx = a.knn_idx;
    double* __restrict__ nrm = a.nrm; double* __restrict__ nrm_sorted = a.nrm_sorted; TargetRec* __restrict__ rec = a.rec;
    const int k = a.k;
    if (bx == 0 && threadIdx.x < 4) a.list_counts[threadIdx.x] = 0u;
    const uint32_t spos = xcd_block(bx, nbx) * QN_BLOCK + threadIdx.x;
    if (spos >= a.n) return;
    const uint32_t i = __float_as_uint(a.sorted[spos].w);
    const int32_t* nb = knn_idx + (size_t)i * k;
    int found = 0;
    double mean[3] = {0, 0, 0};
    double nv[3] = {0, 0, 0};
    auto store = [&]() __attribute__((always_inline)) {
#pragma unroll
      for (int u = 0; u < 3; u++) nrm[(size_t)i * 3 + u] = nv[u];
      if (nrm_sorted) {
#pragma unroll
        for (int u = 0; u < 3; u++) nrm_sorted[(size_t)spos * 3 + u] = nv[u];
      }
      if (rec) { TargetRec r; r.p = raw[i];
#pragma unroll
        for (int u = 0; u < 3; u++) { r.n[u] = nv[u]; r.pad[u] = 0; }
        rec[i] = r; }
    };
    double c[6] = {0, 0, 0, 0, 0, 0};
    if (k <= QN_COV_REG) {
      int32_t u[QN_COV_REG]; float4 q[QN_COV_REG];
      static_assert(QN_COV_REG % 4 == 0, "the index row is fetched four entries at a time");
      if ((k & 3) == 0) {
        const int4* __restrict__ nb4 = (const int4*)nb;
#pragma unroll
        for (int e = 0; e < QN_COV_REG; e += 4) {
          const int4 v = e < k ? nb4[e >> 2] : make_int4(-1, -1, -1, -1);
          u[e] = v.x; u[e + 1] = v.y; u[e + 2] = v.z; u[e + 3] = v.w;
        }
      } else {
#pragma unroll
        for (int e = 0; e < QN_COV_REG; e++) u[e] = e < k ? nb[e] : -1;
      }
#pragma unroll
      for (int e = 0; e < QN_COV_REG; e++) q[e] = raw[u[e] < 0 ? 0 : u[e]];
#pragma unroll
      for (int e = 0; e < QN_COV_REG; e++) if (u[e] >= 0) { mean[0] += (double)q[e].x; mean[1] += (double)q[e].y; mean[2] += (double)q[e].z; found++; }
      if (found == 0) { store(); return; }
      mean[0] /= found; mean[1] /= found; mean[2] /= found;
#pragma unroll
      for (int e = 0; e < QN_COV_REG; e++) if (u[e] >= 0) {
        const double dx = (double)q[e].x - mean[0], dy = (double)q[e].y - mean[1], dz = (double)q[e].z - mean[2];
        c[0] += dx * dx; c[1] += dx * dy; c[2] += dx * dz; c[3] += dy * dy; c[4] += dy * dz; c[5] += dz * dz;
      }
    } else {
    for (int j = 0; j < k; j += QN_COV_BATCH) {
      int32_t u[QN_COV_BATCH]; float4 q[QN_COV_BATCH];
#pragma unroll
      for (int e = 0; e < QN_COV_BATCH; e++) u[e] = j + e < k ? nb[j + e] : -1;
#pragma unroll
      for (int e = 0; e < QN_COV_BATCH; e++) q[e] = raw[u[e] < 0 ? 0 : u[e]];
#pragma unroll
      for (int e = 0; e < QN_COV_BATCH; e++) if (u[e] >= 0) { mean[0] += (double)q[e].x; mean[1] += (double)q[e].y; mean[2] += (double)q[e].z; found++; }
    }
    if (found == 0) { store(); return; }
    mean[0] /= found; mean[1] /= found; mean[2] /= found;
    for (int j = 0; j < k; j += QN_COV_BATCH) {
      int32_t u[QN_COV_BATCH]; float4 q[QN_COV_BATCH];
#pragma unroll
      for (int e = 0; e < QN_COV_BATCH; e++) u[e] = j + e < k ? nb[j + e] : -1;
#pragma unroll
      for (int e = 0; e < QN_COV_BATCH; e++) q[e] = raw[u[e] < 0 ? 0 : u[e]];
#pragma unroll
      for (int e = 0; e < QN_COV_BATCH; e++) if (u[e] >= 0) {
        const double dx = (double)q[e].x - mean[0], dy = (double)q[e].y - mean[1], dz = (double)q[e].z - mean[2];
        c[0] += dx * dx; c[1] += dx * dy; c[2] += dx * dz; c[3] += dy * dy; c[4] += dy * dz; c[5] += dz * dz;
      }
    }
    }
#pragma unroll
    for (int t = 0; t < 6; t++) c[t] /= found;
    double w[3], V[3][3];
    sym_eig3(c, w, V);
    nv[0] = V[0][2]; nv[1] = V[1][2]; nv[2] = V[2][2];
    store();
  }
};
static __global__ void __launch_bounds__(QN_BLOCK) k_cov_from_idx(const float4* __restrict__ raw, const float4* __restrict__ sorted, uint32_t n, int k, const int32_t* __restrict__ knn_idx, double* __restrict__ nrm,
                                                                  double* __restrict__ nrm_sorted, TargetRec* __restrict__ rec, uint32_t* __restrict__ list_counts) {
  const CovFromIdxK::Args a{raw, sorted, n, k, knn_idx, nrm, nrm_sorted, rec, list_counts};
  CovFromIdxK::run(a, blockIdx.x, gridDim.x);
}

static __global__ void k_cov_from_normals(const double* __restrict__ nrm, uint32_t n, double* __restrict__ cov6) {
  const uint32_t i = blockIdx.x * blockDim.x + threadIdx.x;
  if (i >= n) return;
  const double a = nrm[(size_t)i * 3], b = nrm[(size_t)i * 3 + 1], c = nrm[(size_t)i * 3 + 2];
  double* o = cov6 + (size_t)i * 6;
  o[0] = 1.0 - 0.999 * a * a; o[1] = -0.999 * a * b; o[2] = -0.999 * a * c; o[3] = 1.0 - 0.999 * b * b; o[4] = -0.999 * b * c; o[5] = 1.0 - 0.999 * c * c;
}


#ifndef QN_KNN_BLOCK
#define QN_KNN_BLOCK 64
#endif
struct KnnHistArgs { GridView g; int k; float r0; int max_rounds; int32_t* knn_idx; float* knn_d2; uint2* fb_list; uint32_t* fb_count; uint2* gen_list; uint32_t* gen_count; };
__device__ __forceinline__ float late_s(float v) { asm volatile("" : "+s"(v)); return v; }
template <bool LIST, int HCAP, bool MM = true>
struct KnnHistK {
  static constexpr int TB = QN_KNN_BLOCK, OCC = HCAP <= 32 ? 4 : 3;
  using Args = KnnHistArgs;
  static __device__ __forceinline__ void run(const Args& a, const uint32_t bx, const uint32_t nbx) {
    __shared__ WaveLdsH<HCAP> lds[QN_KNN_BLOCK / 64];
    const GridView g = grid_resolve(a.g);
    const int k = a.k, max_rounds = a.max_rounds;
    int32_t* __restrict__ knn_idx = a.knn_idx; float* __restrict__ knn_d2 = a.knn_d2;
    uint2* __restrict__ fb_list = a.fb_list; uint32_t* __restrict__ fb_count = a.fb_count; uint2* __restrict__ gen_list = a.gen_list; uint32_t* __restrict__ gen_count = a.gen_count;
    float r0 = a.r0; if (r0 < 0.f) r0 = -r0 * g.cell;
    r0 = uni(r0);
    WaveLdsH<HCAP>* my = &lds[threadIdx.x >> 6];
    const uint32_t nq = LIST ? uni(*fb_count) : g.n;
    if (LIST && g.dbg && bx == 0 && threadIdx.x == 0) atomicAdd(&g.dbg[4], nq);
    const uint32_t wave0 = (LIST ? bx : xcd_block(bx, nbx)) * (QN_KNN_BLOCK / 64) + (threadIdx.x >> 6), nwaves = nbx * (QN_KNN_BLOCK / 64);
    for (uint32_t base = wave0 * 16; base < nq; base += nwaves * 16) {
      const uint32_t slot = base + (threadIdx.x & 15);
      bool active = slot < nq;
      uint32_t t = slot; float r = r0; bool general = false;
      if (LIST && active) { const uint2 rec = fb_list[slot]; t = rec.x; r = __uint_as_float(rec.y & 0x7fffffffu); general = (rec.y >> 31) != 0; }
      const float4 q = active ? g.pts[t] : make_float4(0, 0, 0, 0);
      const uint32_t i = __float_as_uint(q.w);
      int status = 2;
      {
        const int st = wave_knn_hist<HCAP, MM>(g, q.x, q.y, q.z, active && !general, r, k, max_rounds < 0 ? -max_rounds : max_rounds, my, knn_idx, knn_d2, i);
        if (!general) status = st;
      }
      if (!active || (threadIdx.x & 63) >= 16 || status == 0) continue;
      if (LIST) { const uint32_t fs = atomicAdd(gen_count, 1u); gen_list[fs] = make_uint2(t, __float_as_uint(r)); }
      else if (status == 2 || r > 2.5f * late_s(r0) || max_rounds < 0 ) { const uint32_t fs = atomicAdd(gen_count, 1u); gen_list[fs] = make_uint2(t, __float_as_uint(r)); }
      else { const uint32_t fs = atomicAdd(fb_count, 1u); fb_list[fs] = make_uint2(t, __float_as_uint(r)); }
    }
  }
};
template <bool LIST, int HCAP, bool MM = true>
__global__ void __launch_bounds__(QN_KNN_BLOCK, HCAP <= 32 ? 4 : 3) k_knn_hist(GridView g, int k, float r0, int max_rounds, int32_t* __restrict__ knn_idx, float* __restrict__ knn_d2,
                                                       uint2* __restrict__ fb_list, uint32_t* __restrict__ fb_count, uint2* __restrict__ gen_list, uint32_t* __restrict__ gen_count) {
  const KnnHistArgs a{g, k, r0, max_rounds, knn_idx, knn_d2, fb_list, fb_count, gen_list, gen_count};
  KnnHistK<LIST, HCAP, MM>::run(a, blockIdx.x, gridDim.x);
}

struct KnnSingleK {
  static constexpr int TB = QN_BLOCK, OCC = 1;
  struct Args { GridView g; int k; int32_t* knn_idx; float* knn_d2; const uint2* list; const uint32_t* count; uint2* gen_list; uint32_t* gen_count; };
  static __device__ __forceinline__ void run(const Args& a, const uint32_t bx, const uint32_t nbx) {
    __shared__ WaveLdsH1 lds[QN_BLOCK / 64];
    const GridView g = grid_resolve(a.g);
    const int k = a.k;
    int32_t* __restrict__ knn_idx = a.knn_idx; float* __restrict__ knn_d2 = a.knn_d2; const uint2* __restrict__ list = a.list; uint2* __restrict__ gen_list = a.gen_list; uint32_t* __restrict__ gen_count = a.gen_count;
    WaveLdsH1* my = &lds[threadIdx.x >> 6];
    const uint32_t nq = uni(*a.count);
    if (g.dbg && bx == 0 && threadIdx.x == 0) atomicAdd(&g.dbg[8], nq);
    const uint32_t wave0 = bx * (QN_BLOCK / 64) + (threadIdx.x >> 6), nwaves = nbx * (QN_BLOCK / 64);
    for (uint32_t e = wave0; e < nq; e += nwaves) {
      const uint2 rec = list[e];
      const float4 q = g.pts[rec.x];
      const uint32_t i = __float_as_uint(q.w);
      const int st = wave_knn_single(g, q.x, q.y, q.z, __uint_as_float(rec.y & 0x7fffffffu), k, my, knn_idx + (size_t)i * k, knn_d2 ? knn_d2 + (size_t)i * k : nullptr);
      if (st != 0 && (threadIdx.x & 63) == 0) { if (g.dbg) atomicAdd(&g.dbg[9], 1u); const uint32_t fs = atomicAdd(gen_count, 1u); gen_list[fs] = make_uint2(rec.x, rec.y & 0x7fffffffu); }
    }
  }
};
static __global__ void __launch_bounds__(QN_BLOCK) k_knn_single(GridView g, int k, int32_t* __restrict__ knn_idx, float* __restrict__ knn_d2,
                                                                const uint2* __restrict__ list, const uint32_t* __restrict__ count, uint2* __restrict__ gen_list, uint32_t* __restrict__ gen_count) {
  const KnnSingleK::Args a{g, k, knn_idx, knn_d2, list, count, gen_list, gen_count};
  KnnSingleK::run(a, blockIdx.x, gridDim.x);
}

template <int MODE>
__device__ __forceinline__ void xform_query(const float Tf[12], float x, float y, float z, float& qx, float& qy, float& qz) {
  if (MODE == 0) {
    qx = ((Tf[0] * x + Tf[1] * y) + Tf[2] * z) + Tf[3];
    qy = ((Tf[4] * x + Tf[5] * y) + Tf[6] * z) + Tf[7];
    qz = ((Tf[8] * x + Tf[9] * y) + Tf[10] * z) + Tf[11];
  } else {
    qx = Tf[0] * x + (Tf[1] * y + (Tf[2] * z + Tf[3]));
    qy = Tf[4] * x + (Tf[5] * y + (Tf[6] * z + Tf[7]));
    qz = Tf[8] * x + (Tf[9] * y + (Tf[10] * z + Tf[11]));
  }
}

__device__ __forceinline__ uint32_t late(uint32_t v) { asm volatile("" : "+v"(v)); return v; }
template <int MODE>
__device__ __forceinline__ void store_nn(unsigned long long key, uint32_t i, uint32_t t, double thr2, int32_t* __restrict__ corr, float* __restrict__ sqd, int32_t* __restrict__ nn_idx) {
  const float d2 = key_d2(key);
  if (MODE == 0) nn_idx[t] = key != QN_INF_KEY ? (int32_t)key_idx(key) : -1;
  if (MODE == 0) {
    const bool found = key != QN_INF_KEY;
    sqd[i] = found ? d2 : 0.f;
    corr[i] = (found && (double)d2 < thr2) ? (int32_t)key_idx(key) : -1;
  } else {
    sqd[i] = key != QN_INF_KEY ? d2 : __int_as_float(0x7f800000);
  }
}

struct NnOpt { float4* clear_ref; int cond; int group, group_min; unsigned long long* probe; uint32_t fb_small; };
struct NnSearchArgs { GridView src, tgt; const GicpState* st; double thr2; float r0; int max_rounds; int32_t* corr; float* sqd; int32_t* nn_idx; float4* nn_ref;
                      uint2* fb_list; uint32_t* fb_count; uint2* big_list; uint32_t* big_count; int big_blocks; float big_ratio; uint32_t* far_stats; NnOpt opt; };
template <int MODE, bool LIST, int BLOCK, bool GROUP = false>
struct NnSearchK {
  static constexpr int TB = BLOCK, OCC = GROUP ? 5 : 6;
  using Args = NnSearchArgs;
  static __device__ __forceinline__ void run(const Args& a, const uint32_t bx, const uint32_t nbx) {
    GridView src = a.src, tgt = a.tgt; const GicpState* __restrict__ st = a.st; const double thr2 = a.thr2; float r0 = a.r0; const int max_rounds = a.max_rounds;
    int32_t* __restrict__ corr = a.corr; float* __restrict__ sqd = a.sqd; int32_t* __restrict__ nn_idx = a.nn_idx; float4* __restrict__ nn_ref = a.nn_ref;
    uint2* __restrict__ fb_list = a.fb_list; uint32_t* __restrict__ fb_count = a.fb_count; uint2* __restrict__ big_list = a.big_list; uint32_t* __restrict__ big_count = a.big_count;
    const int big_blocks = a.big_blocks; const float big_ratio = a.big_ratio; uint32_t* __restrict__ far_stats = a.far_stats; const NnOpt opt = a.opt;

  __shared__ WaveLds lds[BLOCK / 64];
  if (MODE == 0 && uni(st->phase) != 0) return;
  if (MODE == 1 && uni(st->phase) != 2) return;
  if (opt.cond && !(uni(st->reserved) & opt.cond)) return;
  src = grid_resolve(src); tgt = grid_resolve(tgt); if (r0 < 0.f) r0 = -r0 * tgt.cell;
  __shared__ float sTf[12];
  if (threadIdx.x < 12) sTf[threadIdx.x] = (float)st->x0[threadIdx.x];
  __syncthreads();
  if (LIST && (int)bx >= (int)nbx - big_blocks) {
    const uint32_t nbig = uni(*big_count);
    if (tgt.dbg && bx == nbx - 1 && threadIdx.x == 0) atomicAdd(&tgt.dbg[7], nbig);
    uint32_t nfar = 0;
    const uint32_t bw0 = (bx - (nbx - big_blocks)) * (BLOCK / 64) + (threadIdx.x >> 6), nbw = big_blocks * (BLOCK / 64);
    const uint32_t E = (GROUP && opt.group && nbig >= (uint32_t)opt.group_min) ? min(16u, (nbig + (uint32_t)opt.group - 1u) / (uint32_t)opt.group) : 1u;
    if (GROUP && E > 1u) {
      const int lane = threadIdx.x & 63, qs = lane & 15;
      WaveLds* wl = &lds[threadIdx.x >> 6];
      const float INF = __int_as_float(0x7f800000);
      for (uint32_t w0 = bw0 * E; w0 < nbig; w0 += nbw * E) {
        const uint32_t slot = w0 + (uint32_t)qs;
        const bool active = (uint32_t)qs < E && slot < nbig;
        const uint2 rec = active ? big_list[slot] : make_uint2(0u, 0u);
        const float4 p = active ? src.pts[rec.x] : make_float4(0.f, 0.f, 0.f, 0.f);
        float qx, qy, qz; { float Tf[12];
#pragma unroll
          for (int j = 0; j < 12; j++) Tf[j] = sTf[j];
          xform_query<MODE>(Tf, p.x, p.y, p.z, qx, qy, qz); }
        const float v = __uint_as_float(rec.y);
        const float r = v > 0.f ? v * 1.1f + 0.5f * tgt.cell : -v;
        const bool finite_q = (qx - qx == 0.f) && (qy - qy == 0.f) && (qz - qz == 0.f) && (r - r == 0.f);
        unsigned long long key = QN_INF_KEY; float second = INF, d_unseen = INF;
        unsigned long long todo = __ballot(active);
        while (todo) {
// ... 806 lines not shown
```

### fast-lio-sam-qn_amd/csrc/qn_knn_hist.cuh

```cuda
#pragma once
#include "qn_device.cuh"
#include "qn_engine.h"
#include <type_traits>

namespace qn {

#define QN_HB 64
#define QN_HW (QN_HB + 5)
template <int HCAP>
struct WaveLdsH {
  WaveLds s;
  union alignas(16) {
    uint32_t hist[16][QN_HW];
    unsigned long long list[16][HCAP + 1];
    uint4 zero_[(16 * QN_HW + 3) / 4];
  } u;
  uint32_t cnt[16];
  uint32_t kth[16];
  alignas(16) uint32_t tile_sc[64 * 4];
};

typedef float qn_f4v __attribute__((ext_vector_type(4)));
#define QN_MM_FAR 1.0e15f
#define QN_MM_NCH 4
static_assert(QN_MM_NCH == 4, "tile_sc holds 64 x QN_MM_NCH words and is cleared with one 16-byte store per lane; the hit masks are two 32-bit words");
static_assert(QN_CTX_MAX_POINTS <= 0x03ffffffu + 1u, "the 26-bit position field of tile_sc must hold every position of the largest cloud a context takes");
__device__ __forceinline__ uint32_t stage_chunk_mm(const GridView& g, WaveLds* lds, uint32_t* __restrict__ sc_out, const uint32_t cb, const uint32_t total,
                                                   const float Ox, const float Oy, const float Oz, float& c2max, const int j) {
  const int lane = threadIdx.x & 63;
  const uint32_t slot = cb + lane;
  float4 rel = make_float4(QN_MM_FAR, 0.f, 0.f, QN_MM_FAR * QN_MM_FAR); uint32_t sc = 63u << 26;
  if (slot < total) {
    const uint32_t sidx = lds->seg_start[j] + (slot - lds->seg_excl[j]);
    sc = sidx | (lds->seg_cid[j] << 26);
    const float4 p = g.pts[sidx];
    rel.x = p.x - Ox; rel.y = p.y - Oy; rel.z = p.z - Oz; rel.w = (rel.x * rel.x + rel.y * rel.y) + rel.z * rel.z;
    c2max = fmaxf(c2max, rel.w);
  }
  wave_lds_fence();
  lds->tile[lane] = rel; sc_out[lane] = sc;
  wave_lds_fence();
  return min(64u, total - cb);
}

template <int HCAP, bool MM = true>
__device__ __forceinline__ int wave_knn_hist(const GridView& g, float qx, float qy, float qz, bool active, float& r, int k, int max_rounds,
                                             WaveLdsH<HCAP>* L, int32_t* __restrict__ idx_base, float* __restrict__ d2_base, const uint32_t row) {
  const int lane = threadIdx.x & 63, qs = lane & 15, sub = lane >> 4;
  WaveLds* lds = &L->s;
  const int cx = cell_coord(qx, g.ox, g.inv_cell, g.nx);
  const int cy = cell_coord(qy, g.oy, g.inv_cell, g.ny);
  const int cz = cell_coord(qz, g.oz, g.inv_cell, g.nz);
  const float INF = __int_as_float(0x7f800000);
  int status = active ? 1 : 0;
  unsigned long long todo = __ballot(active);
  for (int round = 0; todo != 0 && round < max_rounds; round++) {
    const bool mine = (todo >> lane) & 1ull;
    uint32_t cid; int ncl; uint32_t nseg_all;
    build_clusters<4>(g, lds, todo, cx, cy, cz, qx, qy, qz, r, cid, ncl, nseg_all);
    { uint4* hz = (uint4*)&L->u.hist[0][0];
#pragma unroll
      for (int e = 0; e < (16 * QN_HW + 3) / 4; e += 64) if (e + lane < (16 * QN_HW + 3) / 4) hz[e + lane] = make_uint4(0u, 0u, 0u, 0u); }
    wave_lds_fence();
    const int base = (int)(__float_as_uint(4.f * r * r) >> 20) - (QN_HB - 2);
    const bool one_cluster = ncl == 1;
    const int base1 = mine ? base : -(1 << 28);
    uint32_t ncand;
    float Ox = 0.f, Oy = 0.f, Oz = 0.f, bsel = 0.f, q2 = 0.f, c2max = 0.f;
    if constexpr (MM) {
      const int l0 = __ffsll((long long)todo) - 1;
      Ox = rdlane(qx, l0); Oy = rdlane(qy, l0); Oz = rdlane(qz, l0);
      const float rx = qx - Ox, ry = qy - Oy, rz = qz - Oz;
      q2 = (rx * rx + ry * ry) + rz * rz;
      bsel = sub == 0 ? -2.f * rx : (sub == 1 ? -2.f * ry : (sub == 2 ? -2.f * rz : 1.f));
    }
    const float* tilef = (const float*)&lds->tile[0];
    const qn_f4v cin = {q2, q2, q2, q2};
    auto mm_groups = [&](const float (&av)[4], const uint32_t cnt, auto&& per_group) __attribute__((always_inline)) {
      qn_f4v d = __builtin_amdgcn_mfma_f32_16x16x4f32(av[0], bsel, cin, 0, 0, 0);
#pragma unroll
      for (int gi = 0; gi < 4; gi++) {
        qn_f4v dn = d;
        if (gi < 3) dn = __builtin_amdgcn_mfma_f32_16x16x4f32(av[gi + 1], bsel, cin, 0, 0, 0);
        if ((uint32_t)(16 * gi) < cnt) per_group(gi, d);
        d = dn;
      }
    };
    auto load_av = [&](float (&av)[4]) __attribute__((always_inline)) {
#pragma unroll
      for (int gi = 0; gi < 4; gi++) av[gi] = tilef[(16 * gi + qs) * 4 + sub];
    };
    const bool cached = nseg_all <= 64u && one_cluster;
    float avc[QN_MM_NCH][4];
    if constexpr (MM) {
      auto p1_group = [&](const uint32_t* __restrict__ scb, const int gi, const qn_f4v d) __attribute__((always_inline)) {
        if (one_cluster) {
#pragma unroll
          for (int e = 0; e < 4; e++) {
            const int bin = min(max((__float_as_int(d[e]) >> 20) - base1, 0), QN_HB - 1);
            atomicAdd(&L->u.hist[qs][bin], 1u);
          }
        } else {
          const uint4 cc = *(const uint4*)&scb[16 * gi + 4 * sub];
          const uint32_t ccv[4] = {cc.x >> 26, cc.y >> 26, cc.z >> 26, cc.w >> 26};
#pragma unroll
          for (int e = 0; e < 4; e++) {
            const int bin = max((__float_as_int(d[e]) >> 20) - base, 0);
            const bool ok = mine && ccv[e] == cid && bin < QN_HB - 1;
            atomicAdd(&L->u.hist[qs][ok ? bin : QN_HB + sub], 1u);
          }
        }
      };
      ncand = stream_tables<false>(g, lds, ncl, nseg_all, [&](const uint32_t total) __attribute__((always_inline)) {
        uint32_t cb0 = 0u;
        if (cached) {
          ((uint4*)L->tile_sc)[lane] = make_uint4(0u, 0u, 0u, 0u);
          wave_lds_fence();
          { const uint32_t ex = lds->seg_excl[lane], nx = lane < 63 ? lds->seg_excl[(lane + 1) & 63] : total;
            if (nx > ex && ex < 64u * QN_MM_NCH) L->tile_sc[ex] = (uint32_t)lane + 1u; }
          wave_lds_fence();
          uint32_t carry = 0u;
#pragma unroll
          for (int c = 0; c < QN_MM_NCH; c++) {
            if ((uint32_t)(64 * c) < total) {
              const uint32_t mk = max(wave_incl_max_u32(L->tile_sc[64 * c + lane]), carry);
              carry = rdlane(mk, 63);
              const uint32_t cnt = stage_chunk_mm(g, lds, L->tile_sc + 64 * c, 64u * c, total, Ox, Oy, Oz, c2max, (int)mk - 1);
              load_av(avc[c]);
              mm_groups(avc[c], cnt, [&](const int, const qn_f4v d) __attribute__((always_inline)) {
#pragma unroll
                for (int e = 0; e < 4; e++) atomicAdd(&L->u.hist[qs][min(max((__float_as_int(d[e]) >> 20) - base1, 0), QN_HB - 1)], 1u);
              });
            }
          }
          cb0 = 64u * QN_MM_NCH;
        }
        const uint32_t exs = lds->seg_excl[lane], nxs = lane < 63 ? lds->seg_excl[(lane + 1) & 63] : total;
        for (uint32_t cb = cb0; cb < total; cb += 64) {
          const int jg = chunk_segment(lds->tile_cid, cb, exs, nxs);
          const uint32_t cnt = stage_chunk_mm(g, lds, lds->tile_cid, cb, total, Ox, Oy, Oz, c2max, jg);
          float av[4]; load_av(av);
          mm_groups(av, cnt, [&](const int gi, const qn_f4v d) __attribute__((always_inline)) { p1_group(lds->tile_cid, gi, d); });
        }
      });
    } else {
    auto bin_of = [&](const float4& cp) __attribute__((always_inline)) { return max((int)(__float_as_uint(sqdist(qx, qy, qz, cp.x, cp.y, cp.z)) >> 20) - base, 0); };
    ncand = one_cluster
      ? stream_clusters<4>(g, lds, ncl, nseg_all, [&](const float4& cp, bool, uint32_t) __attribute__((always_inline)) {
          const int bin = min(max((int)(__float_as_uint(sqdist(qx, qy, qz, cp.x, cp.y, cp.z)) >> 20) - base1, 0), QN_HB - 1);
          atomicAdd(&L->u.hist[qs][bin], 1u);
        })
      : stream_clusters<4>(g, lds, ncl, nseg_all, [&](const float4& cp, bool in_tile, uint32_t ccid) __attribute__((always_inline)) {
          const int bin = bin_of(cp);
          const bool ok = mine && in_tile && ccid == cid && bin < QN_HB - 1;
          atomicAdd(&L->u.hist[qs][ok ? bin : QN_HB + sub], 1u);
        });
    }
    wave_lds_fence();
    uint32_t hv[16], mysum = 0;
#pragma unroll
    for (int j = 0; j < 16; j++) { hv[j] = L->u.hist[qs][sub * 16 + j]; if (j == 15 && sub == 3) hv[j] = 0u; mysum += hv[j]; }
    const uint32_t s0 = __shfl(mysum, qs), s1 = __shfl(mysum, qs + 16), s2 = __shfl(mysum, qs + 32), s3 = __shfl(mysum, qs + 48);
    uint32_t run = (sub > 0 ? s0 : 0u) + (sub > 1 ? s1 : 0u) + (sub > 2 ? s2 : 0u);
    const bool enough = s0 + s1 + s2 + s3 >= (uint32_t)k;
    int cross = 1 << 20;
#pragma unroll
    for (int j = 0; j < 16; j++) { run += hv[j]; if (cross == (1 << 20) && run >= (uint32_t)k) cross = sub * 16 + j; }
    cross = min(cross, __shfl_xor(cross, 16)); cross = min(cross, __shfl_xor(cross, 32));
    const uint32_t tau_bits = (uint32_t)(base + cross + 1) << 20;
    wave_lds_fence();
    if (lane < 16) { L->cnt[lane] = 0; L->kth[lane] = 0x7f800000u; }
    { uint4* lz = (uint4*)&L->u.list[0][0];
      constexpr int NZ = (int)(sizeof(L->u.list) / 16);
      static_assert(sizeof(L->u.list) % 16 == 0, "list rows are cleared with 16-byte stores");
#pragma unroll
      for (int e = 0; e < NZ; e += 64) if (e + lane < NZ) lz[e + lane] = make_uint4(0xffffffffu, 0xffffffffu, 0xffffffffu, 0xffffffffu); }
    wave_lds_fence();
    const bool collect = mine && enough;
    if constexpr (MM) {
      const float R2 = wave_max_f(fmaxf(c2max, mine ? q2 : 0.f));
      const float thr = collect ? (__uint_as_float(tau_bits) + 2.f * (R2 * 1.52587890625e-5f)) * 1.000001f : -__int_as_float(0x7f800000);
      float dummy = 0.f;
      const uint32_t cidm = cid;
      if (cached) {
        uint32_t mw[QN_MM_NCH / 2] = {0u, 0u};
#pragma unroll
        for (int c = 0; c < QN_MM_NCH; c++) {
          uint32_t& m = mw[c >> 1];
          if ((uint32_t)(64 * c) < ncand) {
            const uint32_t cnt = min(64u, ncand - 64u * c);
            qn_f4v d = __builtin_amdgcn_mfma_f32_16x16x4f32(avc[c][0], bsel, cin, 0, 0, 0);
#pragma unroll
            for (int gi = 0; gi < 4; gi++) {
              qn_f4v dn = d;
              if (gi < 3) dn = __builtin_amdgcn_mfma_f32_16x16x4f32(avc[c][gi + 1], bsel, cin, 0, 0, 0);
#pragma unroll
              for (int e = 0; e < 4; e++) m = __builtin_amdgcn_alignbit(m, __float_as_uint(d[e] - thr), 31);
              d = dn;
            }
          } else m <<= 16;
        }
        const uint32_t cntl = (uint32_t)(__popc(mw[0]) + __popc(mw[1]));
        const uint32_t h0 = __shfl(cntl, qs), h1 = __shfl(cntl, qs + 16), h2 = __shfl(cntl, qs + 32), h3 = __shfl(cntl, qs + 48);
        uint32_t pos = (sub > 0 ? h0 : 0u) + (sub > 1 ? h1 : 0u) + (sub > 2 ? h2 : 0u);
        if (sub == 0) L->cnt[qs] = h0 + h1 + h2 + h3;
        while (__any((mw[0] | mw[1]) != 0u)) {
          const bool lo = mw[0] != 0u;
          uint32_t w = lo ? mw[0] : mw[1];
          if (w != 0u) {
            const uint32_t I = (uint32_t)__clz((int)w);
            const uint32_t at = (lo ? 0u : 128u) + ((I >> 4) << 6) + (((I >> 2) & 3u) << 4) + 4u * (uint32_t)sub + (I & 3u);
            if (pos < HCAP) L->u.list[qs][pos] = (unsigned long long)(L->tile_sc[at] & 0x03ffffffu);
            pos++;
            w &= ~(0x80000000u >> I);
            if (lo) mw[0] = w; else mw[1] = w;
          }
        }
        wave_lds_fence();
      }
      if (!cached || ncand > 64u * QN_MM_NCH) {
      stream_tables<true>(g, lds, ncl, nseg_all, [&](const uint32_t total) __attribute__((always_inline)) {
        const uint32_t exs = lds->seg_excl[lane], nxs = lane < 63 ? lds->seg_excl[(lane + 1) & 63] : total;
        for (uint32_t cb = cached ? 64u * QN_MM_NCH : 0u; cb < total; cb += 64) {
          const int jg = chunk_segment(lds->tile_cid, cb, exs, nxs);
          const uint32_t cnt = stage_chunk_mm(g, lds, lds->tile_cid, cb, total, Ox, Oy, Oz, dummy, jg);
          float av[4]; load_av(av);
          mm_groups(av, cnt, [&](const int gi, const qn_f4v d) __attribute__((always_inline)) {
            bool hit[4];
#pragma unroll
            for (int e = 0; e < 4; e++) hit[e] = d[e] < thr;
            const uint4 cc = *(const uint4*)&lds->tile_cid[16 * gi + 4 * sub];
            if (!one_cluster) { hit[0] = hit[0] && (cc.x >> 26) == cidm; hit[1] = hit[1] && (cc.y >> 26) == cidm; hit[2] = hit[2] && (cc.z >> 26) == cidm; hit[3] = hit[3] && (cc.w >> 26) == cidm; }
            const uint32_t scv[4] = {cc.x, cc.y, cc.z, cc.w};
            if (hit[0] || hit[1] || hit[2] || hit[3]) {
#pragma unroll
              for (int e = 0; e < 4; e++) if (hit[e]) {
                const uint32_t pos = atomicAdd(&L->cnt[qs], 1u);
                if (pos < HCAP) L->u.list[qs][pos] = (unsigned long long)(scv[e] & 0x03ffffffu);
              }
            }
          });
        }
      }, ncand);
      }
      wave_lds_fence();
      const uint32_t Pn = min(L->cnt[qs], (uint32_t)HCAP);
      const int pmax = wave_max_i(collect ? (int)Pn : 0);
#pragma unroll
      for (int j = 0; j < HCAP / 4; j++) {
        if (4 * j >= pmax) break;
        const uint32_t slot = (uint32_t)(sub + 4 * j);
        if (collect && slot < Pn) {
          const float4 p = g.pts[(uint32_t)L->u.list[qs][slot]];
          L->u.list[qs][slot] = pack_key(sqdist(qx, qy, qz, p.x, p.y, p.z), __float_as_uint(p.w));
        }
      }
    } else {
    auto collect_one = [&](const float4& cp) __attribute__((always_inline)) {
      const float d2 = sqdist(qx, qy, qz, cp.x, cp.y, cp.z);
      if (collect && __float_as_uint(d2) < tau_bits) {
        const uint32_t pos = atomicAdd(&L->cnt[qs], 1u);
        if (pos < HCAP) L->u.list[qs][pos] = pack_key(d2, __float_as_uint(cp.w));
      }
    };
    if (one_cluster) stream_clusters<4, true>(g, lds, ncl, nseg_all, [&](const float4& cp, bool, uint32_t) __attribute__((always_inline)) { collect_one(cp); }, ncand);
    else stream_clusters<4, true>(g, lds, ncl, nseg_all, [&](const float4& cp, bool in_tile, uint32_t ccid) __attribute__((always_inline)) { if (in_tile && ccid == cid) collect_one(cp); }, ncand);
    }
    wave_lds_fence();
    const uint32_t P = L->cnt[qs];
    const bool ok = collect && P <= HCAP;
    const int maxP = wave_max_i(ok ? (int)P : 0);
    unsigned long long own[HCAP / 4]; int rank[HCAP / 4];
#pragma unroll
    for (int j = 0; j < HCAP / 4; j++) { own[j] = L->u.list[qs][sub + 4 * j]; rank[j] = 0; }
    auto rank_pass = [&](auto NJ) __attribute__((always_inline)) {
      for (int f = 0; f < maxP; f += 4) {
        unsigned long long kf[4];
#pragma unroll
        for (int u = 0; u < 4; u++) kf[u] = L->u.list[qs][min(f + u, HCAP)];
#pragma unroll
        for (int u = 0; u < 4; u++) {
#pragma unroll
          for (int j = 0; j < decltype(NJ)::value; j++) rank[j] += kf[u] < own[j] ? 1 : 0;
        }
      }
    };
    if (HCAP > 32 && maxP > 32) rank_pass(std::integral_constant<int, HCAP / 4>());
    else if (maxP > 28) rank_pass(std::integral_constant<int, 8>());
    else if (maxP > 24) rank_pass(std::integral_constant<int, 7>());
    else rank_pass(std::integral_constant<int, 6>());
#pragma unroll
    for (int j = 0; j < HCAP / 4; j++) if (own[j] != QN_INF_KEY && rank[j] == k - 1) L->kth[qs] = (uint32_t)(own[j] >> 32);
    wave_lds_fence();
    const float kth_d2 = __uint_as_float(L->kth[qs]);
    if (g.dbg && lane == 0) { atomicAdd(&g.dbg[0], (uint32_t)ncl); atomicAdd(&g.dbg[1], ncand); }
    bool retry = false;
    if (mine) {
      const int* b = lds->box[cid];
      const int ex0 = b[0], ex1 = b[1], ey0 = b[2], ey1 = b[3], ez0 = b[4], ez1 = b[5];
      float d = INF;
      if (ex0 > 0) d = fminf(d, qx - (g.ox + ex0 * g.cell));
      if (ex1 < g.nx - 1) d = fminf(d, (g.ox + (ex1 + 1) * g.cell) - qx);
      if (ey0 > 0) d = fminf(d, qy - (g.oy + ey0 * g.cell));
      if (ey1 < g.ny - 1) d = fminf(d, (g.oy + (ey1 + 1) * g.cell) - qy);
      if (ez0 > 0) d = fminf(d, qz - (g.oz + ez0 * g.cell));
      if (ez1 < g.nz - 1) d = fminf(d, (g.oz + (ez1 + 1) * g.cell) - qz);
      const bool whole = d == INF || !(r == r);
      if (!enough) {
        if (whole) status = 2;
        else {
          const uint32_t tot = s0 + s1 + s2 + s3;
          if (4u * tot < (uint32_t)k) {
            int kk = k; asm volatile("" : "+s"(kk));
            r = tot > 0 ? 2.f * r * sqrtf((float)kk / (float)tot) * 1.1f : 4.f * r + g.cell;
          } else { r = 2.f * r + g.cell; retry = true; }
        }
      } else if (!ok) status = 2;
      else {
        d -= g.eps;
        if (whole || (d > 0.f && kth_d2 < d * d)) {
          status = 0;
          uint32_t row_l = row; asm volatile("" : "+v"(row_l));
          int32_t* __restrict__ idx_out = idx_base + (size_t)row_l * k; float* __restrict__ d2_out = d2_base ? d2_base + (size_t)row_l * k : nullptr;
#pragma unroll
          for (int j = 0; j < HCAP / 4; j++) if (own[j] != QN_INF_KEY && rank[j] < k) {
            idx_out[rank[j]] = (int32_t)key_idx(own[j]);
            if (d2_out) d2_out[rank[j]] = key_d2(own[j]);
          }
        } else { r = fmaxf(sqrtf(kth_d2) * 1.000001f + g.eps, r + g.eps); retry = true; }
      }
    }
    todo = __ballot(retry && round + 1 < max_rounds);
    if (g.dbg && lane == 0 && todo) atomicAdd(&g.dbg[3], (uint32_t)__popcll(todo));
  }
  return status;
}


#define QN_HCAP1 128
struct WaveLdsH1 {
  WaveLds s;
  uint32_t hist[QN_HB];
  unsigned long long list[QN_HCAP1];
  uint32_t cnt, kth;
  unsigned long long best;
  uint32_t second, pad;
};

__device__ __forceinline__ int wave_knn_single(const GridView& g, float qx, float qy, float qz, float r, int k, WaveLdsH1* L,
                                               int32_t* __restrict__ idx_out, float* __restrict__ d2_out) {
  const int lane = threadIdx.x & 63;
  const float INF = __int_as_float(0x7f800000);
  if (!(qx == qx) || !(qy == qy) || !(qz == qz) || !(r == r)) return 2;
  const CapBox cap = cap_of(g, qx, qy, qz);
  if (cap.S > 0.f) r = fmaxf(r, sqrtf(cap.S) + 0.5f * g.cell);
  const float r_in = r;
  for (int round = 0; round < 64; round++) {
    const float rx = cap_extent(g, cap, r, 0), ry = cap_extent(g, cap, r, 1), rz = cap_extent(g, cap, r, 2);
    int x0 = rfl(cell_coord(qx - rx, g.ox, g.inv_cell, g.nx)), x1 = rfl(cell_coord(qx + rx, g.ox, g.inv_cell, g.nx));
    int y0 = rfl(cell_coord(qy - ry, g.oy, g.inv_cell, g.ny)), y1 = rfl(cell_coord(qy + ry, g.oy, g.inv_cell, g.ny));
    int z0 = rfl(cell_coord(qz - rz, g.oz, g.inv_cell, g.nz)), z1 = rfl(cell_coord(qz + rz, g.oz, g.inv_cell, g.nz));
    const bool tile_mode = ((x1 >> 3) - (x0 >> 3) + 1) * (y1 - y0 + 1) * (z1 - z0 + 1) > 128;
    if (tile_mode) {
      x0 = (x0 >> 3) << 3; x1 = min(((x1 >> 3) << 3) + 7, g.nx - 1);
      y0 = (y0 >> 2) << 2; y1 = min(((y1 >> 2) << 2) + 3, g.ny - 1);
      z0 = (z0 >> 2) << 2; z1 = min(((z1 >> 2) << 2) + 3, g.nz - 1);
    }
    wave_lds_fence();
    L->hist[lane] = 0; if (lane == 0) { L->cnt = 0; L->kth = 0x7f800000u; }
    wave_lds_fence();
    const int base = (int)(__float_as_uint(4.f * r * r) >> 20) - (QN_HB - 2);
    stream_box(g, x0, x1, y0, y1, z0, z1, tile_mode, &L->s, [&](const float4& p, bool valid, uint32_t) __attribute__((always_inline)) {
      const int bin = max((int)(__float_as_uint(sqdist(qx, qy, qz, p.x, p.y, p.z)) >> 20) - base, 0);
      if (valid && bin < QN_HB - 1) atomicAdd(&L->hist[bin], 1u);
    });
    wave_lds_fence();
    const uint32_t hv = lane < QN_HB - 1 ? L->hist[lane] : 0u;
    const uint32_t cum = wave_incl_scan_u32(hv, lane);
    const uint32_t total = rdlane(cum, 63);
    const bool enough = total >= (uint32_t)k;
    const unsigned long long reach = __ballot(cum >= (uint32_t)k);
    const int cross = reach ? __ffsll((long long)reach) - 1 : QN_HB - 2;
    uint32_t tau_bits = (uint32_t)(base + cross + 1) << 20;
    if (enough && rdlane(cum, cross) > (uint32_t)QN_HCAP1 && cross > 0) {
      const uint32_t below = rdlane(cum, cross - 1), need = (uint32_t)k - below;
      const uint32_t hi20 = (uint32_t)(base + cross);
      wave_lds_fence();
      L->hist[lane] = 0;
      wave_lds_fence();
      stream_box(g, x0, x1, y0, y1, z0, z1, tile_mode, &L->s, [&](const float4& p, bool valid, uint32_t) __attribute__((always_inline)) {
        const uint32_t bits = __float_as_uint(sqdist(qx, qy, qz, p.x, p.y, p.z));
        if (valid && (bits >> 20) == hi20) atomicAdd(&L->hist[(bits >> 14) & 63u], 1u);
      });
      wave_lds_fence();
      const uint32_t cum2 = wave_incl_scan_u32(L->hist[lane], lane);
      const unsigned long long reach2 = __ballot(cum2 >= need);
      const int sub = reach2 ? __ffsll((long long)reach2) - 1 : 63;
      tau_bits = (hi20 << 20) + ((uint32_t)(sub + 1) << 14);
    }
    float d = INF;
    if (x0 > 0) d = fminf(d, cap_face_dist(cap, qx - (g.ox + x0 * g.cell), 0));
    if (x1 < g.nx - 1) d = fminf(d, cap_face_dist(cap, (g.ox + (x1 + 1) * g.cell) - qx, 0));
    if (y0 > 0) d = fminf(d, cap_face_dist(cap, qy - (g.oy + y0 * g.cell), 1));
    if (y1 < g.ny - 1) d = fminf(d, cap_face_dist(cap, (g.oy + (y1 + 1) * g.cell) - qy, 1));
    if (z0 > 0) d = fminf(d, cap_face_dist(cap, qz - (g.oz + z0 * g.cell), 2));
    if (z1 < g.nz - 1) d = fminf(d, cap_face_dist(cap, (g.oz + (z1 + 1) * g.cell) - qz, 2));
    const bool whole = d == INF;
    if (!enough) {
      if (whole) return 2;
      if (r_in > 6.f * g.cell) r += (1.f + round) * g.cell;
      else r = total > 0 ? fmaxf(2.f * r * sqrtf((float)k / (float)total) * 1.1f, r + g.cell) : 2.f * r + g.cell;
      continue;
    }
    stream_box(g, x0, x1, y0, y1, z0, z1, tile_mode, &L->s, [&](const float4& p, bool valid, uint32_t) __attribute__((always_inline)) {
      const float d2 = sqdist(qx, qy, qz, p.x, p.y, p.z);
      if (valid && __float_as_uint(d2) < tau_bits) {
        const uint32_t pos = atomicAdd(&L->cnt, 1u);
        if (pos < QN_HCAP1) L->list[pos] = pack_key(d2, __float_as_uint(p.w));
      }
    });
    wave_lds_fence();
    const uint32_t P = L->cnt;
    if (P > QN_HCAP1) return 2;
    const unsigned long long own0 = (uint32_t)lane < P ? L->list[lane] : QN_INF_KEY, own1 = (uint32_t)lane + 64u < P ? L->list[lane + 64] : QN_INF_KEY;
    int rank0 = 0, rank1 = 0;
    for (uint32_t f = 0; f < P; f++) { const unsigned long long kf = L->list[f]; rank0 += kf < own0 ? 1 : 0; rank1 += kf < own1 ? 1 : 0; }
    if (own0 != QN_INF_KEY && rank0 == k - 1) L->kth = (uint32_t)(own0 >> 32);
    if (own1 != QN_INF_KEY && rank1 == k - 1) L->kth = (uint32_t)(own1 >> 32);
    wave_lds_fence();
    const float kth_d2 = __uint_as_float(L->kth);
    const float df = d - g.eps;
    if (whole || (df > 0.f && kth_d2 < df * df)) {
      if (own0 != QN_INF_KEY && rank0 < k) { idx_out[rank0] = (int32_t)key_idx(own0); if (d2_out) d2_out[rank0] = key_d2(own0); }
      if (own1 != QN_INF_KEY && rank1 < k) { idx_out[rank1] = (int32_t)key_idx(own1); if (d2_out) d2_out[rank1] = key_d2(own1); }
      if (lane == 0) { L->second = 0x7f800000u; }
      wave_lds_fence();
      if (own0 != QN_INF_KEY && rank0 == 0) L->best = own0;
      if (own1 != QN_INF_KEY && rank1 == 0) L->best = own1;
      if (own0 != QN_INF_KEY && rank0 == 1) L->second = (uint32_t)(own0 >> 32);
      if (own1 != QN_INF_KEY && rank1 == 1) L->second = (uint32_t)(own1 >> 32);
      wave_lds_fence();
      return 0;
    }
    r = fmaxf(sqrtf(kth_d2) * 1.000001f + g.eps, r + g.eps);
  }
  return 2;
}

}
```

### fast-lio-sam-qn_amd/csrc/qn_knn_kernels.cuh

```cuda
#pragma once
#include "qn_device.cuh"
#ifndef QN_BLOCK
#define QN_BLOCK 256
#endif

namespace qn {

template <int KMAX>
__device__ __forceinline__ void store_knn(const BestK<KMAX>& sink, int32_t* __restrict__ knn_idx, float* __restrict__ knn_d2) {
  const int k = sink.k;
#pragma unroll
  for (int j = 0; j < KMAX; j++) if (j >= KMAX - k) {
    const bool ok = sink.a[j] != QN_INF_KEY;
    knn_idx[j - (KMAX - k)] = ok ? (int32_t)key_idx(sink.a[j]) : -1;
    if (knn_d2) knn_d2[j - (KMAX - k)] = ok ? key_d2(sink.a[j]) : 0.f;
  }
}

struct KnnCovArgs { GridView g; const float4* raw; int k; float r0; int max_rounds; double* cov; int32_t* knn_idx; float* knn_d2; uint2* fb_list; uint32_t* fb_count; };
template <int KMAX, bool LIST, int S>
struct KnnCovK {
  static constexpr int TB = QN_BLOCK, OCC = 3;
  using Args = KnnCovArgs;
  static __device__ __forceinline__ void run(const Args& a, const uint32_t bx, const uint32_t nbx) {
    const GridView g = grid_resolve(a.g);
    const int k = a.k, max_rounds = a.max_rounds; float r0 = a.r0;
    int32_t* __restrict__ knn_idx = a.knn_idx; float* __restrict__ knn_d2 = a.knn_d2; uint2* __restrict__ fb_list = a.fb_list; uint32_t* __restrict__ fb_count = a.fb_count;

  __shared__ WaveLdsK lds[QN_BLOCK / 64];
  if (r0 < 0.f) r0 = -r0 * g.cell;
  WaveLdsK* my = &lds[threadIdx.x >> 6];
  const uint32_t nq = LIST ? uni(*fb_count) : g.n;
  if (LIST && g.dbg && bx == 0 && threadIdx.x == 0) atomicAdd(&g.dbg[4], nq);
  const uint32_t wave0 = bx * (QN_BLOCK / 64) + (threadIdx.x >> 6), nwaves = nbx * (QN_BLOCK / 64);
  constexpr uint32_t QPW = 64 / S;
  for (uint32_t base = wave0 * QPW; base < nq; base += nwaves * QPW) {
    const uint32_t slot = base + (threadIdx.x & (QPW - 1));
    const bool active = slot < nq;
    uint32_t t = slot; float r = r0;
    if (LIST && active) { const uint2 rec = fb_list[slot]; t = rec.x; r = __uint_as_float(rec.y); }
    const float4 q = active ? g.pts[t] : make_float4(0, 0, 0, 0);
    BestK<KMAX> sink; sink.init(k, my->pend, g.dbg);
    float d_unseen;
    const bool cert = wave_search<S>(g, q.x, q.y, q.z, active, r, __int_as_float(0x7f800000), max_rounds, sink, &my->s, d_unseen);
    if (!active || (threadIdx.x & 63) >= QPW) continue;
    const uint32_t i = __float_as_uint(q.w);
    if (cert || LIST) store_knn(sink, knn_idx + (size_t)i * k, knn_d2 ? knn_d2 + (size_t)i * k : nullptr);
    else {
      const uint32_t fs = atomicAdd(fb_count, 1u);
      fb_list[fs] = make_uint2(t, __float_as_uint(r));
    }
  }
  }
};
template <int KMAX, bool LIST, int S>
__global__ void __launch_bounds__(QN_BLOCK, 3) k_knn_cov(GridView g, const float4* __restrict__ raw, int k, float r0, int max_rounds,
                                                      double* __restrict__ cov, int32_t* __restrict__ knn_idx, float* __restrict__ knn_d2,
                                                      uint2* __restrict__ fb_list, uint32_t* __restrict__ fb_count) {
  const KnnCovArgs a{g, raw, k, r0, max_rounds, cov, knn_idx, knn_d2, fb_list, fb_count};
  KnnCovK<KMAX, LIST, S>::run(a, blockIdx.x, gridDim.x);
}

}
```

### fast-lio-sam-qn_amd/qn_amd/engine.py

```python
import ctypes as C
import os
import numpy as np
from . import build as _build

QN_OK, QN_ERR_INVALID_ARG, QN_ERR_EMPTY_CLOUD, QN_ERR_CAPACITY, QN_ERR_NOT_READY, QN_ERR_HIP, QN_ERR_NO_DEVICE = range(7)
QN_SOURCE, QN_TARGET = 0, 1
QN_VERIFY_SRC, QN_VERIFY_DST, QN_VERIFY_COARSE, QN_VERIFY_FINAL = 0, 1, 2, 3
FLOAT_MAX = 3.4028234663852886e38
KERNEL_FAMILIES = ["grid_build", "knn_cov", "nn_search", "nn_fallback", "accumulate", "solve", "fitness", "transform",
                   "fpfh_normals", "fpfh_spfh", "fpfh_fpfh", "feat_match", "gn_tick_fused", "knn_select", "match_tail", "far_refresh", "align_persist"]


class GicpParams(C.Structure):
    _fields_ = [("k_correspondences", C.c_int32), ("max_iterations", C.c_int32), ("max_corr_dist", C.c_double),
                ("transformation_epsilon", C.c_double), ("rotation_epsilon", C.c_double), ("optimizer", C.c_int32),
                ("lm_max_iterations", C.c_int32), ("lm_init_lambda_factor", C.c_double), ("force_iterations", C.c_int32),
                ("ransac_iterations", C.c_int32), ("ransac_outlier_threshold", C.c_double),
                ("euclidean_fitness_epsilon", C.c_double)]


class GicpResult(C.Structure):
    _fields_ = [("T", C.c_float * 16), ("T64", C.c_double * 16), ("H", C.c_double * 36), ("fitness", C.c_double),
                ("iterations", C.c_int32), ("converged", C.c_int32), ("lm_failed", C.c_int32), ("reserved", C.c_int32)]

# ... 162 lines not shown
        self.p.lm_max_iterations = n; self._push()

    def setLMInitLambdaFactor(self, f):
        self.p.lm_init_lambda_factor = f; self._push()

    def setOptimizer(self, name):
        self.p.optimizer = 0 if name == "lm" else 1; self._push()

    def setForceIterations(self, n):
        self.p.force_iterations = n; self._push()

    def setInputSource(self, xyz):
        a, n, stride = _cloud_arg(xyz); self._n[0] = n
        st = self._l.qn_gicp_set_source(self.ctx.h, _p(a), C.c_uint32(n), C.c_uint32(stride))
        if st != QN_ERR_EMPTY_CLOUD:
            self.ctx.check(st)

    def setInputTarget(self, xyz):
        a, n, stride = _cloud_arg(xyz); self._n[1] = n
        st = self._l.qn_gicp_set_target(self.ctx.h, _p(a), C.c_uint32(n), C.c_uint32(stride))
        if st != QN_ERR_EMPTY_CLOUD:
            self.ctx.check(st)

    def setInputSourceDevice(self, ptr, n, stride):
        self._n[0] = n
        self.ctx.check(self._l.qn_gicp_set_source_device(self.ctx.h, C.c_void_p(ptr), C.c_uint32(n), C.c_uint32(stride)))

    def setInputTargetDevice(self, ptr, n, stride):
        self._n[1] = n
        self.ctx.check(self._l.qn_gicp_set_target_device(self.ctx.h, C.c_void_p(ptr), C.c_uint32(n), C.c_uint32(stride)))

    def calculateSourceCovariances(self):
        return self._l.qn_gicp_compute_covariances(self.ctx.h, C.c_int(QN_SOURCE)) == QN_OK

    def calculateTargetCovariances(self):
        return self._l.qn_gicp_compute_covariances(self.ctx.h, C.c_int(QN_TARGET)) == QN_OK

    def align(self, guess=None):
        res = GicpResult()
        g = None if guess is None else np.ascontiguousarray(guess, dtype=np.float32)
        st = self._l.qn_gicp_align(self.ctx.h, None if g is None else _p(g), C.byref(res))
        if st in (QN_ERR_EMPTY_CLOUD, QN_ERR_NOT_READY):
            self._res = None
            return None
        self.ctx.check(st)
        self._res = res
        return res

    def alignedCloud(self):
        out = np.zeros((self._n[0], 4), dtype=np.float32)
        self.ctx.check(self._l.qn_gicp_transformed_source(self.ctx.h, _p(out), C.c_uint32(16)))
        return out[:, :3]

    def getFitnessScore(self, max_range=1.7976931348623157e308):
        if self._res is None:
            return 1.7976931348623157e308
        if max_range >= 1.7976931348623157e308:
            return self._res.fitness
        s = C.c_double()
        self.ctx.check(self._l.qn_gicp_fitness(self.ctx.h, C.c_double(max_range), C.byref(s)))
        return s.value

    def hasConverged(self):
        return bool(self._res.converged) if self._res is not None else False

    def getFinalTransformation(self):
        return np.array(self._res.T, dtype=np.float32).reshape(4, 4) if self._res is not None else np.eye(4, dtype=np.float32)

    def result_dict(self):
        r = self._res
        return dict(T=np.array(r.T64).reshape(4, 4), Tf=np.array(r.T, dtype=np.float32).reshape(4, 4), H=np.array(r.H).reshape(6, 6),
                    fitness=r.fitness, iterations=r.iterations, converged=bool(r.converged), lm_failed=bool(r.lm_failed),
                    trace=self.trace())

    def trace(self):
        buf = (IterTrace * 1024)(); n = C.c_uint32()
        self.ctx.check(self._l.qn_gicp_get_trace(self.ctx.h, buf, C.c_uint32(1024), C.byref(n)))
        return np.array([[t.y0, t.lambda_, t.rho, t.max_dR, t.max_dt, t.inner, t.accepted] for t in buf[:n.value]]).reshape(-1, 7)

    def covariances(self, which):
        out = np.zeros((self._n[which], 3, 3))
        self.ctx.check(self._l.qn_gicp_get_covariances(self.ctx.h, C.c_int(which), _p(out)))
        return out

    def knn(self, which, k):
        idx = np.zeros((self._n[which], k), dtype=np.int32); d2 = np.zeros((self._n[which], k), dtype=np.float32)
        self.ctx.check(self._l.qn_gicp_knn(self.ctx.h, C.c_int(which), C.c_int(k), _p(idx), _p(d2)))
        return idx, d2

    def linearize(self, T):
        T = np.ascontiguousarray(T, dtype=np.float64)
        H = np.zeros((6, 6)); b = np.zeros(6); e = C.c_double()
        corr = np.zeros(self._n[0], dtype=np.int32); sqd = np.zeros(self._n[0], dtype=np.float32)
        self.ctx.check(self._l.qn_gicp_linearize(self.ctx.h, _p(T), _p(H), _p(b), C.byref(e), _p(corr), _p(sqd)))
        return H, b, e.value, corr, sqd

    def compute_error(self, T):
        T = np.ascontiguousarray(T, dtype=np.float64); e = C.c_double()
        self.ctx.check(self._l.qn_gicp_compute_error(self.ctx.h, _p(T), C.byref(e)))
        return e.value


class _ParamsScope:

    def __init__(self, ctx):
        self.ctx = ctx; self.saved = GicpParams()
        ctx.check(ctx._l.qn_gicp_get_params(ctx.h, C.byref(self.saved)))

    def __enter__(self):
        return self

    def __exit__(self, *exc):
        self.ctx.check(self.ctx._l.qn_gicp_set_params(self.ctx.h, C.byref(self.saved)))
        return False


def _reference_gicp(ctx, k, max_iter, max_corr_dist, trans_eps):
    p = GicpParams(); ctx._l.qn_gicp_default_params(C.byref(p))
    p.k_correspondences, p.max_iterations, p.max_corr_dist, p.transformation_epsilon = k, max_iter, max_corr_dist, trans_eps
    ctx.check(ctx._l.qn_gicp_set_params(ctx.h, C.byref(p)))


def icp_alignment(ctx, src, dst, *, k=15, max_iter=32, max_corr_dist=52.5, trans_eps=0.01, score_thr=1.5):
    a, ns, stride = _cloud_arg(src); b, nt, _ = _cloud_arg(dst)
    res = GicpResult(); valid = C.c_int()
    with _ParamsScope(ctx):
        _reference_gicp(ctx, k, max_iter, max_corr_dist, trans_eps)
        st = ctx._l.qn_icp_alignment(ctx.h, _p(a), C.c_uint32(ns), _p(b), C.c_uint32(nt), C.c_uint32(stride),
                                     C.c_double(score_thr), C.byref(res), C.byref(valid))
    if st == QN_ERR_EMPTY_CLOUD:
        return dict(valid=False, converged=False, score=1.7976931348623157e308, T=np.eye(4), iterations=0)
    ctx.check(st)
    return dict(valid=bool(valid.value), converged=bool(res.converged), score=res.fitness,
                T=np.array(res.T, dtype=np.float32).reshape(4, 4).astype(np.float64), iterations=res.iterations)


def fpfh(ctx, xyz):
    a, n, stride = _cloud_arg(xyz)
    out = np.zeros((n, 33), dtype=np.float32)
    ctx.check(ctx._l.qn_fpfh(ctx.h, _p(a), C.c_uint32(n), C.c_uint32(stride), _p(out)))
    return out


def match_optimized(ctx, src, dst, fs, ft, thr_dist=35.0, num_max_corres=200, tuple_scale=0.95):
    a, ns, stride = _cloud_arg(src); b, nt, _ = _cloud_arg(dst)
    fs = np.ascontiguousarray(fs, dtype=np.float32); ft = np.ascontiguousarray(ft, dtype=np.float32)
    pairs = np.zeros((num_max_corres, 2), dtype=np.int32); n = C.c_uint32()
    ctx.check(ctx._l.qn_match_optimized(ctx.h, _p(a), C.c_uint32(ns), _p(b), C.c_uint32(nt), C.c_uint32(stride), _p(fs), _p(ft),
                                        C.c_float(thr_dist), C.c_int(num_max_corres), C.c_float(tuple_scale), _p(pairs), C.c_uint32(num_max_corres), C.byref(n)))
    return pairs[:min(n.value, num_max_corres)].copy()


class QuatroParams(C.Structure):
    _fields_ = [("fpfh_normal_radius", C.c_double), ("fpfh_radius", C.c_double), ("noise_bound", C.c_double),
                ("rot_gnc_factor", C.c_double), ("rot_cost_diff_thr", C.c_double), ("rot_max_iter", C.c_int32),
                ("estimate_scale", C.c_int32), ("use_optimized_matching", C.c_int32), ("distance_threshold", C.c_double),
                ("max_num_corres", C.c_int32), ("rng_seed", C.c_uint32), ("tuple_scale", C.c_double)]


def quatro_default_params():
    p = QuatroParams(); lib().qn_quatro_default_params(C.byref(p)); return p


class Quatro:

    def __init__(self, ctx, fpfh_normal_radius=0.9, fpfh_radius=1.5, noise_bound=0.3, rot_gnc_factor=1.4, rot_cost_diff_thr=1e-4,
# ... 759 lines not shown
```

### include/qn_engine.h

```cpp
#ifndef QN_ENGINE_H
#define QN_ENGINE_H

#include <stdint.h>

#ifdef __cplusplus
extern "C" {
#endif

typedef struct qn_ctx qn_ctx;

enum {
  QN_OK = 0,
  QN_ERR_INVALID_ARG = 1,
  QN_ERR_EMPTY_CLOUD = 2,
  QN_ERR_CAPACITY = 3,
  QN_ERR_NOT_READY = 4,
  QN_ERR_HIP = 5,
  QN_ERR_NO_DEVICE = 6
};

enum { QN_SOURCE = 0, QN_TARGET = 1 };
enum { QN_OPT_LM = 0, QN_OPT_GN = 1 };

typedef struct {
// ... 199 lines not shown
int  qn_kf_overlap_points(qn_kf_store*, uint32_t pair_slot, int dir, float* nn_d2_out, int32_t* nn_idx_out);
#define QN_RANGE_MAX_ROWS 1024
#define QN_RANGE_MAX_COLS 8192
typedef struct qn_range_params { uint32_t n_rows, n_cols; double el_lo, el_hi, min_range; uint32_t window_rows, window_cols; double tol_abs, tol_rel; } qn_range_params;
typedef struct qn_freespace_dir { uint32_t n, n_finite, in_fov, observed, seen_through, occluded, agree, reserved; } qn_freespace_dir;
typedef struct qn_freespace { qn_freespace_dir q_in_c, c_in_q; } qn_freespace;
int  qn_kf_range_set_params(qn_kf_store*, const qn_range_params*);
int  qn_kf_range_get_params(qn_kf_store*, qn_range_params*);
int  qn_kf_range_describe(qn_kf_store*, const int32_t* ids, uint32_t count, int* status);
int  qn_kf_range_get(qn_kf_store*, int32_t id, float* near_out , float* far_out);
int  qn_kf_freespace_batch(qn_kf_store*, const int32_t* query, const int32_t* cand, const double* T16 , uint32_t n_pairs,
                           qn_freespace* out, int* status);
int  qn_kf_freespace_points(qn_kf_store*, uint32_t pair_slot, int dir, uint8_t* class_out );
int  qn_kf_add_xyzi(qn_kf_store*, const float* pts, uint32_t n, uint32_t stride_bytes, uint32_t intensity_offset_bytes, int32_t* id_out);
int  qn_kf_build_map(qn_kf_store*, const int32_t* ids, const double* poses16, uint32_t count, double leaf,
                     const float** d_xyzi_out , uint32_t* n_out);
int  qn_kf_download_map(qn_kf_store*, void* out, uint32_t stride_bytes, uint32_t intensity_offset_bytes);
typedef struct qn_static_params { uint32_t min_see_through, agree_weight; } qn_static_params;
void qn_static_default_params(qn_static_params* p);
int  qn_kf_static_classify(qn_kf_store*, const int32_t* ids, const double* poses16, uint32_t count, const uint32_t* wit_off , const uint32_t* wit,
                           const qn_static_params* params, uint32_t* removed_per_entry, int* status);
int  qn_kf_static_points(qn_kf_store*, uint32_t entry, uint8_t* seen_through_out, uint8_t* agree_out, uint8_t* removed_out);
int  qn_kf_build_map_static(qn_kf_store*, double leaf, const float** d_xyzi_out , uint32_t* n_out);
int  qn_loop_candidates(const double* pos_xyz, const double* stamps, uint32_t n, uint32_t query, double radius, double tdiff,
                        uint32_t max_k, int32_t* out, uint32_t* n_out);

int  qn_kf_add_device(qn_kf_store*, const float* d_pts, uint32_t n, uint32_t stride_bytes, int32_t intensity_offset_bytes, int32_t* id_out);
int  qn_kf_download_keyframe(qn_kf_store*, int32_t id, float* xyzi_out );

enum { QN_SIM_GROUND = 0, QN_SIM_WALL = 1, QN_SIM_POLE = 2, QN_SIM_BOX = 3 };
#define QN_SIM_MAX_PRIMS 4096u
#define QN_SIM_MAX_RAYS (1u << 20)
#define QN_SIM_MAX_SCANS 65535u
#define QN_SIM_MAX_TOTAL_RAYS (1ull << 27)
typedef struct {
  uint32_t kind;
  uint32_t pad_;
  double p[6];
} qn_sim_prim;
typedef struct {
  uint32_t n_beams, n_cols;
  const double *cos_el, *sin_el;
  const double *cos_az, *sin_az;
  double min_range, max_range, sigma;
} qn_sim_sensor;
int  qn_sim_lidar_to_store(qn_kf_store*, const qn_sim_prim* prims, uint32_t n_prims, const qn_sim_sensor* sensor, const double* poses16,
                           const uint32_t* seeds, uint32_t n_scans, int32_t* ids_out, uint32_t* n_out);

#define QN_SC_MAX_RINGS 64u
#define QN_SC_MAX_SECTORS 360u
#define QN_SC_MAX_BINS 8192u
#define QN_SC_MAX_PREFILTER 1024u
#define QN_SC_MAX_TOP_K 1024u
#define QN_SC_MAX_RESULTS (1u << 26)
typedef struct {
  uint32_t n_rings;
  uint32_t n_sectors;
  double max_radius;
  double lidar_height;
  uint32_t ringkey_prefilter;
  uint32_t pad_;
} qn_sc_params;
int  qn_kf_sc_set_params(qn_kf_store*, const qn_sc_params* p);
int  qn_kf_sc_get_params(qn_kf_store*, qn_sc_params* p);
int  qn_kf_sc_describe(qn_kf_store*, const int32_t* ids, uint32_t count);
int  qn_kf_sc_get(qn_kf_store*, int32_t id, float* desc , double* ringkey , double* colnorm );
int  qn_kf_sc_query(qn_kf_store*, const int32_t* query_ids, uint32_t nq, const double* stamps, uint32_t n_stamps, double tdiff, uint32_t top_k,
                    int32_t* ids_out, double* dist_out, int32_t* shift_out, uint32_t* n_out);

int  qn_gicp_get_covariances(qn_ctx*, int which, double* cov9_out);
int  qn_gicp_knn(qn_ctx*, int which, int k, int32_t* idx_out, float* d2_out);
int  qn_gicp_linearize(qn_ctx*, const double T[16], double H[36], double b[6], double* err,
                       int32_t* corr_out, float* sqd_out);
int  qn_gicp_compute_error(qn_ctx*, const double T[16], double* err);

int  qn_prof_enable(qn_ctx*, int on);
int  qn_prof_reset(qn_ctx*);
int  qn_prof_get(qn_ctx*, int kernel_family, qn_kernel_stat* out);
int  qn_debug_set(qn_ctx*, const char* key, double value);
int  qn_debug_get_counters(qn_ctx*, uint32_t out[16]);
int  qn_debug_selftest(qn_ctx*, uint32_t n_waves, uint32_t seed, uint32_t* mismatches);
int  qn_debug_get(qn_ctx*, const char* key, double* value);
int  qn_debug_get_grid(qn_ctx*, int which, double out[8]);
int  qn_debug_get_partials(qn_ctx*, double* out, uint32_t* rows_per_buffer, double* state);
int  qn_debug_get_list_probe(qn_ctx*, unsigned long long* out );
int  qn_debug_get_persist_clk(qn_ctx*, unsigned long long* out );
int  qn_debug_get_clk(qn_ctx*, unsigned long long* out , uint32_t* n);

#ifdef __cplusplus
}
#endif
#endif
```

Before: 4435.

## Store kNN tables in sorted-point order and gather covariances from sorted cloud

Adds a pos_of map from original point index to its slot in the cell-sorted array, written during scatter and stable-cell passes. kNN kernels now write rows by sorted position and store neighbour indices as sorted slots, and the covariance kernel gathers neighbours from the sorted array instead of the raw cloud. The aim is more coalesced row writes and more cache-local neighbour gathers in covariance estimation. In exchange it adds a pos_of lookup per stored neighbour, and host read-back needs a remapping kernel with temporary allocations. It also adds a debug accessor for normals.

```diff
diff --git a/fast-lio-sam-qn_amd/csrc/qn_context.h b/fast-lio-sam-qn_amd/csrc/qn_context.h
--- a/fast-lio-sam-qn_amd/csrc/qn_context.h
+++ b/fast-lio-sam-qn_amd/csrc/qn_context.h
@@ -11,6 +11,7 @@
   float4* sorted = nullptr;
   float4* sorted_tmp = nullptr;
   uint32_t* cell_of_pt = nullptr;
+  uint32_t* pos_of = nullptr;
   uint32_t* cell_start = nullptr;
   uint32_t* counts = nullptr;
   double* nrm = nullptr;
diff --git a/fast-lio-sam-qn_amd/csrc/qn_device.cuh b/fast-lio-sam-qn_amd/csrc/qn_device.cuh
--- a/fast-lio-sam-qn_amd/csrc/qn_device.cuh
+++ b/fast-lio-sam-qn_amd/csrc/qn_device.cuh
@@ -24,6 +24,7 @@
   int ntx, nty, ntz;
   uint32_t n;
   const GridDims* dims;
+  const uint32_t* pos_of;
 };
 __device__ __forceinline__ int uni(int v) { return __builtin_amdgcn_readfirstlane(v); }
 __device__ __forceinline__ uint32_t uni(uint32_t v) { return (uint32_t)__builtin_amdgcn_readfirstlane((int)v); }
diff --git a/fast-lio-sam-qn_amd/csrc/qn_engine.hip b/fast-lio-sam-qn_amd/csrc/qn_engine.hip
--- a/fast-lio-sam-qn_amd/csrc/qn_engine.hip
+++ b/fast-lio-sam-qn_amd/csrc/qn_engine.hip
@@ -82,6 +82,7 @@
   sl.take(b.sorted, sizeof(float4) * c->max_points);
   sl.take(b.sorted_tmp, sizeof(float4) * c->max_points);
   sl.take(b.cell_of_pt, sizeof(uint32_t) * c->max_points);
+  sl.take(b.pos_of, sizeof(uint32_t) * c->max_points);
   sl.take(b.cell_start, sizeof(uint32_t) * ((size_t)c->max_cells + 1));
   sl.take(b.counts, sizeof(uint32_t) * ((size_t)c->max_cells + 1));
   sl.take(b.nrm, sizeof(double) * 3 * c->max_points);
@@ -277,7 +278,7 @@
   const uint32_t n = b.n;
   GridView& g = b.grid;
   memset(&g, 0, sizeof(g));
-  g.pts = b.sorted; g.cell_start = b.cell_start; g.dbg = c->dbg_counters; g.n = n; g.dims = b.dims;
+  g.pts = b.sorted; g.cell_start = b.cell_start; g.dbg = c->dbg_counters; g.n = n; g.dims = b.dims; g.pos_of = b.pos_of;
   GridLaunch L;
   L.nb = (n + QN_BLOCK - 1) / QN_BLOCK;
   L.scan_nb = (c->max_cells + QN_BLOCK * QN_SCAN_ITEMS - 1) / (QN_BLOCK * QN_SCAN_ITEMS);
@@ -287,8 +288,8 @@
   L.count = CellCountK::Args{b.raw, n, g, b.counts, b.cell_of_pt};
   L.scan = ScanLookbackK::Args{b.counts, b.dims, b.cell_start, c->scan_status, c->build_epoch, n};
   L.stable = c->stable_cells;
-  L.scat = ScatterK::Args{b.raw, n, b.cell_of_pt, b.cell_start, b.counts, L.stable ? b.sorted_tmp : b.sorted};
-  L.stab = StableCellsK::Args{b.sorted_tmp, n, b.cell_of_pt, b.cell_start, b.sorted};
+  L.scat = ScatterK::Args{b.raw, n, b.cell_of_pt, b.cell_start, b.counts, L.stable ? b.sorted_tmp : b.sorted, L.stable ? (uint32_t*)nullptr : b.pos_of};
+  L.stab = StableCellsK::Args{b.sorted_tmp, n, b.cell_of_pt, b.cell_start, b.sorted, b.pos_of};
   b.has_grid = true; b.has_cov = false; b.knn_tab = nullptr;
   return L;
 }
@@ -299,8 +300,8 @@
     hipLaunchKernelGGL(k_pack_bbox_dims, dim3(L.pack_nb), dim3(QN_BLOCK), 0, s, L.pack.in, L.pack.stride, L.pack.n, L.pack.raw, L.pack.acc, L.pack.max_cells, L.pack.cell_override, L.pack.dims_dev, L.pack.dims_host);
     hipLaunchKernelGGL(k_cell_count, dim3(L.nb), dim3(QN_BLOCK), 0, s, L.count.pts, L.count.n, L.count.g, L.count.counts, L.count.cell_of_pt);
     hipLaunchKernelGGL(k_scan_lookback, dim3(L.scan_nb), dim3(QN_BLOCK), 0, s, L.scan.in, L.scan.dims, L.scan.out, L.scan.status, L.scan.epoch, L.scan.total);
-    hipLaunchKernelGGL(k_scatter, dim3(L.nb), dim3(QN_BLOCK), 0, s, L.scat.pts, L.scat.n, L.scat.cell_of_pt, L.scat.cell_start, L.scat.counts, L.scat.sorted);
-    if (L.stable) hipLaunchKernelGGL(k_stable_cells, dim3(L.nb), dim3(QN_BLOCK), 0, s, L.stab.in, L.stab.n, L.stab.cell_of_pt, L.stab.cell_start, L.stab.out); }
+    hipLaunchKernelGGL(k_scatter, dim3(L.nb), dim3(QN_BLOCK), 0, s, L.scat.pts, L.scat.n, L.scat.cell_of_pt, L.scat.cell_start, L.scat.counts, L.scat.sorted, L.scat.pos_of);
+    if (L.stable) hipLaunchKernelGGL(k_stable_cells, dim3(L.nb), dim3(QN_BLOCK), 0, s, L.stab.in, L.stab.n, L.stab.cell_of_pt, L.stab.cell_start, L.stab.out, L.stab.pos_of); }
   HIPCHK(c, hipGetLastError());
   return QN_OK;
 }
@@ -376,7 +377,7 @@
   L.tail_nb = std::min<uint32_t>((b.n + 63) / 64, lanes ? 64 : 1024);
   L.tail = KnnCovArgs{b.grid, b.raw, k, r0, 64, b.nrm, kidx, kd2, c->fb_list, c->fb_count2 + 2};
   L.cov_nb = (b.n + QN_BLOCK - 1) / QN_BLOCK;
-  L.cov = CovFromIdxK::Args{b.raw, b.sorted, b.n, k, kidx, b.nrm, &b == &c->cloud[0] ? c->nrm_s_sorted : (double*)nullptr, &b == &c->cloud[0] ? (TargetRec*)nullptr : c->tgt_rec, c->fb_count2};
+  L.cov = CovFromIdxK::Args{b.sorted, b.n, k, kidx, b.nrm, &b == &c->cloud[0] ? c->nrm_s_sorted : (double*)nullptr, &b == &c->cloud[0] ? (TargetRec*)nullptr : c->tgt_rec, c->fb_count2};
   return L;
 }
 template <int KMAX>
@@ -393,7 +394,7 @@
     else hipLaunchKernelGGL(HIP_KERNEL_NAME(k_knn_hist<true, HCAP>), dim3(L.lst_nb), dim3(QN_KNN_BLOCK), 0, s, L.lst.g, L.lst.k, L.lst.r0, L.lst.max_rounds, L.lst.knn_idx, L.lst.knn_d2, L.lst.fb_list, L.lst.fb_count, L.lst.gen_list, L.lst.gen_count);
     hipLaunchKernelGGL(k_knn_single, dim3(L.single_nb), dim3(QN_BLOCK), 0, s, L.single.g, L.single.k, L.single.knn_idx, L.single.knn_d2, L.single.list, L.single.count, L.single.gen_list, L.single.gen_count);
     hipLaunchKernelGGL(HIP_KERNEL_NAME(k_knn_cov<KMAX, true, 4>), dim3(L.tail_nb), dim3(QN_BLOCK), 0, s, L.tail.g, L.tail.raw, L.tail.k, L.tail.r0, L.tail.max_rounds, L.tail.cov, L.tail.knn_idx, L.tail.knn_d2, L.tail.fb_list, L.tail.fb_count);
-    hipLaunchKernelGGL(k_cov_from_idx, dim3(L.cov_nb), dim3(QN_BLOCK), 0, s, L.cov.raw, L.cov.sorted, L.cov.n, L.cov.k, L.cov.knn_idx, L.cov.nrm, L.cov.nrm_sorted, L.cov.rec, L.cov.list_counts);
+    hipLaunchKernelGGL(k_cov_from_idx, dim3(L.cov_nb), dim3(QN_BLOCK), 0, s, L.cov.sorted, L.cov.n, L.cov.k, L.cov.knn_idx, L.cov.nrm, L.cov.nrm_sorted, L.cov.rec, L.cov.list_counts);
     return;
   }
   const float r0 = knn_first_radius(c, b);
@@ -404,7 +405,7 @@
   }
   hipLaunchKernelGGL(HIP_KERNEL_NAME(k_knn_cov<KMAX, true, 4>), dim3(std::min<uint32_t>((b.n + 63) / 64, 512)), dim3(QN_BLOCK), 0, s, b.grid, b.raw, k, r0, 64, b.nrm, kidx, kd2, c->fb_list, c->fb_count2);
   const uint32_t nbp = (b.n + QN_BLOCK - 1) / QN_BLOCK;
-  hipLaunchKernelGGL(k_cov_from_idx, dim3(nbp), dim3(QN_BLOCK), 0, s, b.raw, b.sorted, b.n, k, kidx, b.nrm,
+  hipLaunchKernelGGL(k_cov_from_idx, dim3(nbp), dim3(QN_BLOCK), 0, s, b.sorted, b.n, k, kidx, b.nrm,
                      &b == &c->cloud[0] ? c->nrm_s_sorted : (double*)nullptr, &b == &c->cloud[0] ? (TargetRec*)nullptr : c->tgt_rec, c->fb_count2);
 }
 static void note_knn_table(qn_ctx* c, CloudBuf& b, const int32_t* kidx, int k) {
@@ -976,6 +977,22 @@
   *out = c->lanes[lane];
   return QN_OK;
 }
+static int read_knn_table(qn_ctx* h, const CloudBuf& b, int k, const int32_t* tab, const float* tab_d2, int32_t* idx_out, float* d2_out, hipStream_t s) {
+  const size_t cnt = (size_t)b.n * k;
+  int32_t* d_idx = nullptr; float* d_d2 = nullptr;
+  HIPCHK(h, hipMalloc(&d_idx, sizeof(int32_t) * cnt));
+  hipError_t e = (tab_d2 && d2_out) ? hipMalloc(&d_d2, sizeof(float) * cnt) : hipSuccess;
+  if (e == hipSuccess) {
+    hipLaunchKernelGGL(k_knn_table_to_caller, dim3((uint32_t)((cnt + 255) / 256)), dim3(256), 0, s, b.sorted, b.pos_of, b.n, k, tab, d_d2 ? tab_d2 : (const float*)nullptr, d_idx, d_d2);
+    e = hipGetLastError();
+  }
+  if (e == hipSuccess) e = hipMemcpyAsync(idx_out, d_idx, sizeof(int32_t) * cnt, hipMemcpyDeviceToHost, s);
+  if (e == hipSuccess && d_d2) e = hipMemcpyAsync(d2_out, d_d2, sizeof(float) * cnt, hipMemcpyDeviceToHost, s);
+  if (e == hipSuccess) e = hipStreamSynchronize(s);
+  (void)hipFree(d_idx); (void)hipFree(d_d2);
+  if (e != hipSuccess) { h->set_error("k-NN table read-back", e, __LINE__); return QN_ERR_HIP; }
+  return QN_OK;
+}
 extern "C" int qn_gicp_get_lane_knn(qn_ctx* c, uint32_t lane, int which, int32_t* idx_out, uint32_t* n, int* k) {
   if (c && join_target(c) != QN_OK) return QN_ERR_HIP;
   if (!c || !n || !k || (which != 0 && which != 1)) return QN_ERR_INVALID_ARG;
@@ -987,8 +1004,7 @@
   *n = b.n; *k = b.knn_k;
   if (!idx_out) return QN_OK;
   HIPCHK(c, hipSetDevice(c->device));
-  HIPCHK(c, hipMemcpyAsync(idx_out, b.knn_tab, sizeof(int32_t) * (size_t)b.n * b.knn_k, hipMemcpyDeviceToHost, l->stream));
-  HIPCHK(c, hipStreamSynchronize(l->stream));
+  { const int rc = read_knn_table(c, b, b.knn_k, b.knn_tab, nullptr, idx_out, nullptr, l->stream); if (rc != QN_OK) return rc; }
   return clouds_valid(l);
 }
 extern "C" int qn_gicp_get_lane_covariances(qn_ctx* c, uint32_t lane, int which, double* cov9_out) {
@@ -1015,9 +1031,8 @@
   c->params.k_correspondences = ksave;
   b.has_cov = had && (k == ksave);
   if (rc != QN_OK) return rc;
-  HIPCHK(c, hipMemcpyAsync(idx_out, c->dbg_knn_idx, sizeof(int32_t) * (size_t)b.n * k, hipMemcpyDeviceToHost, c->stream));
-  HIPCHK(c, hipMemcpyAsync(d2_out, c->dbg_knn_d2, sizeof(float) * (size_t)b.n * k, hipMemcpyDeviceToHost, c->stream));
-  HIPCHK(c, hipStreamSynchronize(c->stream));
+  rc = read_knn_table(c, b, k, c->dbg_knn_idx, c->dbg_knn_d2, idx_out, d2_out, c->stream);
+  if (rc != QN_OK) return rc;
   c->prof_collect();
   return clouds_valid(c);
 }
@@ -1245,6 +1260,17 @@
       || hipMemcpy(state, c->state, 2 * sizeof(GicpState), hipMemcpyDeviceToHost) != hipSuccess) return QN_ERR_HIP;
   return QN_OK;
 }
+extern "C" int qn_debug_get_source_normals(qn_ctx* c, double* nrm, double* nrm_sorted, uint32_t* pos_of, uint32_t* sorted_idx) {
+  if (!c || !nrm || !nrm_sorted || !pos_of || !sorted_idx) return QN_ERR_INVALID_ARG;
+  const CloudBuf& b = c->cloud[0];
+  if (!b.has_grid || !b.has_cov) return QN_ERR_NOT_READY;
+  std::vector<float4> pts(b.n);
+  if (hipStreamSynchronize(c->stream) != hipSuccess || hipMemcpy(nrm, b.nrm, sizeof(double) * 3 * b.n, hipMemcpyDeviceToHost) != hipSuccess
+      || hipMemcpy(nrm_sorted, c->nrm_s_sorted, sizeof(double) * 3 * b.n, hipMemcpyDeviceToHost) != hipSuccess || hipMemcpy(pos_of, b.pos_of, sizeof(uint32_t) * b.n, hipMemcpyDeviceToHost) != hipSuccess
+      || hipMemcpy(pts.data(), b.sorted, sizeof(float4) * b.n, hipMemcpyDeviceToHost) != hipSuccess) return QN_ERR_HIP;
+  for (uint32_t t = 0; t < b.n; t++) memcpy(&sorted_idx[t], &pts[t].w, sizeof(uint32_t));
+  return clouds_valid(c);
+}
 extern "C" int qn_debug_get_grid(qn_ctx* c, int which, double out[8]) {
   if (!c || (which != 0 && which != 1) || !c->cloud[which].has_grid) return QN_ERR_INVALID_ARG;
   if (hipStreamSynchronize(c->stream) != hipSuccess || (c->stream2 && hipStreamSynchronize(c->stream2) != hipSuccess)) return QN_ERR_HIP;
diff --git a/fast-lio-sam-qn_amd/csrc/qn_gicp_kernels.cuh b/fast-lio-sam-qn_amd/csrc/qn_gicp_kernels.cuh
--- a/fast-lio-sam-qn_amd/csrc/qn_gicp_kernels.cuh
+++ b/fast-lio-sam-qn_amd/csrc/qn_gicp_kernels.cuh
@@ -226,7 +226,7 @@
 
 struct ScatterK {
   static constexpr int TB = QN_BLOCK, OCC = 1;
-  struct Args { const float4* pts; uint32_t n; const uint32_t* cell_of_pt; const uint32_t* cell_start; uint32_t* counts; float4* sorted; };
+  struct Args { const float4* pts; uint32_t n; const uint32_t* cell_of_pt; const uint32_t* cell_start; uint32_t* counts; float4* sorted; uint32_t* pos_of; };
   static __device__ __forceinline__ void run(const Args& a, const uint32_t bx, const uint32_t) {
     const uint32_t i = bx * QN_BLOCK + threadIdx.x;
     if (i >= a.n) return;
@@ -235,17 +235,18 @@
     float4 p = a.pts[i];
     p.w = __uint_as_float(i);
     a.sorted[slot] = p;
+    if (a.pos_of) a.pos_of[i] = slot;
   }
 };
 static __global__ void __launch_bounds__(QN_BLOCK) k_scatter(const float4* __restrict__ pts, uint32_t n, const uint32_t* __restrict__ cell_of_pt,
-                          const uint32_t* __restrict__ cell_start, uint32_t* __restrict__ counts, float4* __restrict__ sorted) {
-  const ScatterK::Args a{pts, n, cell_of_pt, cell_start, counts, sorted};
+                          const uint32_t* __restrict__ cell_start, uint32_t* __restrict__ counts, float4* __restrict__ sorted, uint32_t* __restrict__ pos_of) {
+  const ScatterK::Args a{pts, n, cell_of_pt, cell_start, counts, sorted, pos_of};
   ScatterK::run(a, blockIdx.x, gridDim.x);
 }
 
 struct StableCellsK {
   static constexpr int TB = QN_BLOCK, OCC = 1;
-  struct Args { const float4* in; uint32_t n; const uint32_t* cell_of_pt; const uint32_t* cell_start; float4* out; };
+  struct Args { const float4* in; uint32_t n; const uint32_t* cell_of_pt; const uint32_t* cell_start; float4* out; uint32_t* pos_of; };
   static __device__ __forceinline__ void run(const Args& a, const uint32_t bx, const uint32_t) {
     const float4* __restrict__ in = a.in; float4* __restrict__ out = a.out;
     const uint32_t t = bx * QN_BLOCK + threadIdx.x;
@@ -253,15 +254,16 @@
     const float4 p = in[t];
     const uint32_t i = __float_as_uint(p.w), c = a.cell_of_pt[i];
     const uint32_t s = a.cell_start[c], e = a.cell_start[c + 1];
-    if (e - s > 256u) { out[t] = p; return; }
+    if (e - s > 256u) { out[t] = p; if (a.pos_of) a.pos_of[i] = t; return; }
     uint32_t rank = 0;
     for (uint32_t u = s; u < e; u++) rank += __float_as_uint(in[u].w) < i ? 1u : 0u;
     out[s + rank] = p;
+    if (a.pos_of) a.pos_of[i] = s + rank;
   }
 };
 static __global__ void __launch_bounds__(QN_BLOCK) k_stable_cells(const float4* __restrict__ in, uint32_t n, const uint32_t* __restrict__ cell_of_pt, const uint32_t* __restrict__ cell_start,
-                                      float4* __restrict__ out) {
-  const StableCellsK::Args a{in, n, cell_of_pt, cell_start, out};
+                                      float4* __restrict__ out, uint32_t* __restrict__ pos_of) {
+  const StableCellsK::Args a{in, n, cell_of_pt, cell_start, out, pos_of};
   StableCellsK::run(a, blockIdx.x, gridDim.x);
 }
 
@@ -271,16 +273,17 @@
 #define QN_COV_REG 20
 struct CovFromIdxK {
   static constexpr int TB = QN_BLOCK, OCC = 1;
-  struct Args { const float4* raw; const float4* sorted; uint32_t n; int k; const int32_t* knn_idx; double* nrm; double* nrm_sorted; TargetRec* rec; uint32_t* list_counts; };
+  struct Args { const float4* sorted; uint32_t n; int k; const int32_t* knn_idx; double* nrm; double* nrm_sorted; TargetRec* rec; uint32_t* list_counts; };
   static __device__ __forceinline__ void run(const Args& a, const uint32_t bx, const uint32_t nbx) {
-    const float4* __restrict__ raw = a.raw; const int32_t* __restrict__ knn_idx = a.knn_idx;
+    const float4* __restrict__ sorted = a.sorted; const int32_t* __restrict__ knn_idx = a.knn_idx;
     double* __restrict__ nrm = a.nrm; double* __restrict__ nrm_sorted = a.nrm_sorted; TargetRec* __restrict__ rec = a.rec;
     const int k = a.k;
     if (bx == 0 && threadIdx.x < 4) a.list_counts[threadIdx.x] = 0u;
     const uint32_t spos = xcd_block(bx, nbx) * QN_BLOCK + threadIdx.x;
     if (spos >= a.n) return;
-    const uint32_t i = __float_as_uint(a.sorted[spos].w);
-    const int32_t* nb = knn_idx + (size_t)i * k;
+    const float4 self = sorted[spos];
+    const uint32_t i = __float_as_uint(self.w);
+    const int32_t* nb = knn_idx + (size_t)spos * k;
     int found = 0;
     double mean[3] = {0, 0, 0};
     double nv[3] = {0, 0, 0};
@@ -291,7 +294,7 @@
 #pragma unroll
         for (int u = 0; u < 3; u++) nrm_sorted[(size_t)spos * 3 + u] = nv[u];
       }
-      if (rec) { TargetRec r; r.p = raw[i];
+      if (rec) { TargetRec r; r.p = make_float4(self.x, self.y, self.z, 1.0f);
 #pragma unroll
         for (int u = 0; u < 3; u++) { r.n[u] = nv[u]; r.pad[u] = 0; }
         rec[i] = r; }
@@ -312,7 +315,7 @@
         for (int e = 0; e < QN_COV_REG; e++) u[e] = e < k ? nb[e] : -1;
       }
 #pragma unroll
-      for (int e = 0; e < QN_COV_REG; e++) q[e] = raw[u[e] < 0 ? 0 : u[e]];
+      for (int e = 0; e < QN_COV_REG; e++) q[e] = sorted[u[e] < 0 ? 0 : u[e]];
 #pragma unroll
       for (int e = 0; e < QN_COV_REG; e++) if (u[e] >= 0) { mean[0] += (double)q[e].x; mean[1] += (double)q[e].y; mean[2] += (double)q[e].z; found++; }
       if (found == 0) { store(); return; }
@@ -328,7 +331,7 @@
 #pragma unroll
       for (int e = 0; e < QN_COV_BATCH; e++) u[e] = j + e < k ? nb[j + e] : -1;
 #pragma unroll
-      for (int e = 0; e < QN_COV_BATCH; e++) q[e] = raw[u[e] < 0 ? 0 : u[e]];
+      for (int e = 0; e < QN_COV_BATCH; e++) q[e] = sorted[u[e] < 0 ? 0 : u[e]];
 #pragma unroll
       for (int e = 0; e < QN_COV_BATCH; e++) if (u[e] >= 0) { mean[0] += (double)q[e].x; mean[1] += (double)q[e].y; mean[2] += (double)q[e].z; found++; }
     }
@@ -339,7 +342,7 @@
 #pragma unroll
       for (int e = 0; e < QN_COV_BATCH; e++) u[e] = j + e < k ? nb[j + e] : -1;
 #pragma unroll
-      for (int e = 0; e < QN_COV_BATCH; e++) q[e] = raw[u[e] < 0 ? 0 : u[e]];
+      for (int e = 0; e < QN_COV_BATCH; e++) q[e] = sorted[u[e] < 0 ? 0 : u[e]];
 #pragma unroll
       for (int e = 0; e < QN_COV_BATCH; e++) if (u[e] >= 0) {
         const double dx = (double)q[e].x - mean[0], dy = (double)q[e].y - mean[1], dz = (double)q[e].z - mean[2];
@@ -355,9 +358,9 @@
     store();
   }
 };
-static __global__ void __launch_bounds__(QN_BLOCK) k_cov_from_idx(const float4* __restrict__ raw, const float4* __restrict__ sorted, uint32_t n, int k, const int32_t* __restrict__ knn_idx, double* __restrict__ nrm,
+static __global__ void __launch_bounds__(QN_BLOCK) k_cov_from_idx(const float4* __restrict__ sorted, uint32_t n, int k, const int32_t* __restrict__ knn_idx, double* __restrict__ nrm,
                                                                   double* __restrict__ nrm_sorted, TargetRec* __restrict__ rec, uint32_t* __restrict__ list_counts) {
-  const CovFromIdxK::Args a{raw, sorted, n, k, knn_idx, nrm, nrm_sorted, rec, list_counts};
+  const CovFromIdxK::Args a{sorted, n, k, knn_idx, nrm, nrm_sorted, rec, list_counts};
   CovFromIdxK::run(a, blockIdx.x, gridDim.x);
 }
 
@@ -369,6 +372,16 @@
   o[0] = 1.0 - 0.999 * a * a; o[1] = -0.999 * a * b; o[2] = -0.999 * a * c; o[3] = 1.0 - 0.999 * b * b; o[4] = -0.999 * b * c; o[5] = 1.0 - 0.999 * c * c;
 }
 
+static __global__ void k_knn_table_to_caller(const float4* __restrict__ sorted, const uint32_t* __restrict__ pos_of, uint32_t n, int k, const int32_t* __restrict__ tab,
+                                             const float* __restrict__ tab_d2, int32_t* __restrict__ idx_out, float* __restrict__ d2_out) {
+  const size_t e = (size_t)blockIdx.x * blockDim.x + threadIdx.x;
+  if (e >= (size_t)n * k) return;
+  const uint32_t i = (uint32_t)(e / (uint32_t)k), j = (uint32_t)(e - (size_t)i * k);
+  const uint32_t t = pos_of[i];
+  const int32_t u = t < n ? tab[(size_t)t * k + j] : -1;
+  idx_out[e] = u >= 0 && (uint32_t)u < n ? (int32_t)__float_as_uint(sorted[u].w) : -1;
+  if (d2_out) d2_out[e] = t < n ? tab_d2[(size_t)t * k + j] : 0.f;
+}
 
 #ifndef QN_KNN_BLOCK
 #define QN_KNN_BLOCK 64
@@ -397,10 +410,9 @@
       uint32_t t = slot; float r = r0; bool general = false;
       if (LIST && active) { const uint2 rec = fb_list[slot]; t = rec.x; r = __uint_as_float(rec.y & 0x7fffffffu); general = (rec.y >> 31) != 0; }
       const float4 q = active ? g.pts[t] : make_float4(0, 0, 0, 0);
-      const uint32_t i = __float_as_uint(q.w);
       int status = 2;
       {
-        const int st = wave_knn_hist<HCAP, MM>(g, q.x, q.y, q.z, active && !general, r, k, max_rounds < 0 ? -max_rounds : max_rounds, my, knn_idx, knn_d2, i);
+        const int st = wave_knn_hist<HCAP, MM>(g, q.x, q.y, q.z, active && !general, r, k, max_rounds < 0 ? -max_rounds : max_rounds, my, knn_idx, knn_d2, t);
         if (!general) status = st;
       }
       if (!active || (threadIdx.x & 63) >= 16 || status == 0) continue;
@@ -432,8 +444,7 @@
     for (uint32_t e = wave0; e < nq; e += nwaves) {
       const uint2 rec = list[e];
       const float4 q = g.pts[rec.x];
-      const uint32_t i = __float_as_uint(q.w);
-      const int st = wave_knn_single(g, q.x, q.y, q.z, __uint_as_float(rec.y & 0x7fffffffu), k, my, knn_idx + (size_t)i * k, knn_d2 ? knn_d2 + (size_t)i * k : nullptr);
+      const int st = wave_knn_single(g, q.x, q.y, q.z, __uint_as_float(rec.y & 0x7fffffffu), k, my, knn_idx + (size_t)rec.x * k, knn_d2 ? knn_d2 + (size_t)rec.x * k : nullptr, g.pos_of);
       if (st != 0 && (threadIdx.x & 63) == 0) { if (g.dbg) atomicAdd(&g.dbg[9], 1u); const uint32_t fs = atomicAdd(gen_count, 1u); gen_list[fs] = make_uint2(rec.x, rec.y & 0x7fffffffu); }
     }
   }
diff --git a/fast-lio-sam-qn_amd/csrc/qn_knn_hist.cuh b/fast-lio-sam-qn_amd/csrc/qn_knn_hist.cuh
--- a/fast-lio-sam-qn_amd/csrc/qn_knn_hist.cuh
+++ b/fast-lio-sam-qn_amd/csrc/qn_knn_hist.cuh
@@ -46,6 +46,7 @@
 template <int HCAP, bool MM = true>
 __device__ __forceinline__ int wave_knn_hist(const GridView& g, float qx, float qy, float qz, bool active, float& r, int k, int max_rounds,
                                              WaveLdsH<HCAP>* L, int32_t* __restrict__ idx_base, float* __restrict__ d2_base, const uint32_t row) {
+  static_assert(HCAP < 64, "rank_pos counts a list entry's rank in its low 6 bits");
   const int lane = threadIdx.x & 63, qs = lane & 15, sub = lane >> 4;
   WaveLds* lds = &L->s;
   const int cx = cell_coord(qx, g.ox, g.inv_cell, g.nx);
@@ -177,6 +178,9 @@
       for (int e = 0; e < NZ; e += 64) if (e + lane < NZ) lz[e + lane] = make_uint4(0xffffffffu, 0xffffffffu, 0xffffffffu, 0xffffffffu); }
     wave_lds_fence();
     const bool collect = mine && enough;
+    uint32_t rank_pos[HCAP / 4];
+#pragma unroll
+    for (int j = 0; j < HCAP / 4; j++) rank_pos[j] = 0u;
     if constexpr (MM) {
       const float R2 = wave_max_f(fmaxf(c2max, mine ? q2 : 0.f));
       const float thr = collect ? (__uint_as_float(tau_bits) + 2.f * (R2 * 1.52587890625e-5f)) * 1.000001f : -__int_as_float(0x7f800000);
@@ -251,8 +255,10 @@
         if (4 * j >= pmax) break;
         const uint32_t slot = (uint32_t)(sub + 4 * j);
         if (collect && slot < Pn) {
-          const float4 p = g.pts[(uint32_t)L->u.list[qs][slot]];
+          const uint32_t at = (uint32_t)L->u.list[qs][slot];
+          const float4 p = g.pts[at];
           L->u.list[qs][slot] = pack_key(sqdist(qx, qy, qz, p.x, p.y, p.z), __float_as_uint(p.w));
+          rank_pos[j] = at << 6;
         }
       }
     } else {
@@ -270,9 +276,9 @@
     const uint32_t P = L->cnt[qs];
     const bool ok = collect && P <= HCAP;
     const int maxP = wave_max_i(ok ? (int)P : 0);
-    unsigned long long own[HCAP / 4]; int rank[HCAP / 4];
-#pragma unroll
-    for (int j = 0; j < HCAP / 4; j++) { own[j] = L->u.list[qs][sub + 4 * j]; rank[j] = 0; }
+    unsigned long long own[HCAP / 4];
+#pragma unroll
+    for (int j = 0; j < HCAP / 4; j++) own[j] = L->u.list[qs][sub + 4 * j];
     auto rank_pass = [&](auto NJ) __attribute__((always_inline)) {
       for (int f = 0; f < maxP; f += 4) {
         unsigned long long kf[4];
@@ -281,7 +287,7 @@
 #pragma unroll
         for (int u = 0; u < 4; u++) {
 #pragma unroll
-          for (int j = 0; j < decltype(NJ)::value; j++) rank[j] += kf[u] < own[j] ? 1 : 0;
+          for (int j = 0; j < decltype(NJ)::value; j++) rank_pos[j] += kf[u] < own[j] ? 1u : 0u;
         }
       }
     };
@@ -290,7 +296,7 @@
     else if (maxP > 24) rank_pass(std::integral_constant<int, 7>());
     else rank_pass(std::integral_constant<int, 6>());
 #pragma unroll
-    for (int j = 0; j < HCAP / 4; j++) if (own[j] != QN_INF_KEY && rank[j] == k - 1) L->kth[qs] = (uint32_t)(own[j] >> 32);
+    for (int j = 0; j < HCAP / 4; j++) if (own[j] != QN_INF_KEY && (int)(rank_pos[j] & 63u) == k - 1) L->kth[qs] = (uint32_t)(own[j] >> 32);
     wave_lds_fence();
     const float kth_d2 = __uint_as_float(L->kth[qs]);
     if (g.dbg && lane == 0) { atomicAdd(&g.dbg[0], (uint32_t)ncl); atomicAdd(&g.dbg[1], ncand); }
@@ -323,9 +329,11 @@
           uint32_t row_l = row; asm volatile("" : "+v"(row_l));
           int32_t* __restrict__ idx_out = idx_base + (size_t)row_l * k; float* __restrict__ d2_out = d2_base ? d2_base + (size_t)row_l * k : nullptr;
 #pragma unroll
-          for (int j = 0; j < HCAP / 4; j++) if (own[j] != QN_INF_KEY && rank[j] < k) {
-            idx_out[rank[j]] = (int32_t)key_idx(own[j]);
-            if (d2_out) d2_out[rank[j]] = key_d2(own[j]);
+          for (int j = 0; j < HCAP / 4; j++) if (own[j] != QN_INF_KEY && (int)(rank_pos[j] & 63u) < k) {
+            const int rk = (int)(rank_pos[j] & 63u);
+            if constexpr (MM) idx_out[rk] = (int32_t)(rank_pos[j] >> 6);
+            else idx_out[rk] = (int32_t)g.pos_of[key_idx(own[j])];
+            if (d2_out) d2_out[rk] = key_d2(own[j]);
           }
         } else { r = fmaxf(sqrtf(kth_d2) * 1.000001f + g.eps, r + g.eps); retry = true; }
       }
@@ -348,7 +356,7 @@
 };
 
 __device__ __forceinline__ int wave_knn_single(const GridView& g, float qx, float qy, float qz, float r, int k, WaveLdsH1* L,
-                                               int32_t* __restrict__ idx_out, float* __restrict__ d2_out) {
+                                               int32_t* __restrict__ idx_out, float* __restrict__ d2_out, const uint32_t* __restrict__ pos_of = nullptr) {
   const int lane = threadIdx.x & 63;
   const float INF = __int_as_float(0x7f800000);
   if (!(qx == qx) || !(qy == qy) || !(qz == qz) || !(r == r)) return 2;
@@ -431,8 +439,8 @@
     const float kth_d2 = __uint_as_float(L->kth);
     const float df = d - g.eps;
     if (whole || (df > 0.f && kth_d2 < df * df)) {
-      if (own0 != QN_INF_KEY && rank0 < k) { idx_out[rank0] = (int32_t)key_idx(own0); if (d2_out) d2_out[rank0] = key_d2(own0); }
-      if (own1 != QN_INF_KEY && rank1 < k) { idx_out[rank1] = (int32_t)key_idx(own1); if (d2_out) d2_out[rank1] = key_d2(own1); }
+      if (own0 != QN_INF_KEY && rank0 < k) { idx_out[rank0] = (int32_t)(pos_of ? pos_of[key_idx(own0)] : key_idx(own0)); if (d2_out) d2_out[rank0] = key_d2(own0); }
+      if (own1 != QN_INF_KEY && rank1 < k) { idx_out[rank1] = (int32_t)(pos_of ? pos_of[key_idx(own1)] : key_idx(own1)); if (d2_out) d2_out[rank1] = key_d2(own1); }
       if (lane == 0) { L->second = 0x7f800000u; }
       wave_lds_fence();
       if (own0 != QN_INF_KEY && rank0 == 0) L->best = own0;
diff --git a/fast-lio-sam-qn_amd/csrc/qn_knn_kernels.cuh b/fast-lio-sam-qn_amd/csrc/qn_knn_kernels.cuh
--- a/fast-lio-sam-qn_amd/csrc/qn_knn_kernels.cuh
+++ b/fast-lio-sam-qn_amd/csrc/qn_knn_kernels.cuh
@@ -7,12 +7,12 @@
 namespace qn {
 
 template <int KMAX>
-__device__ __forceinline__ void store_knn(const BestK<KMAX>& sink, int32_t* __restrict__ knn_idx, float* __restrict__ knn_d2) {
+__device__ __forceinline__ void store_knn(const BestK<KMAX>& sink, int32_t* __restrict__ knn_idx, float* __restrict__ knn_d2, const uint32_t* __restrict__ pos_of) {
   const int k = sink.k;
 #pragma unroll
   for (int j = 0; j < KMAX; j++) if (j >= KMAX - k) {
     const bool ok = sink.a[j] != QN_INF_KEY;
-    knn_idx[j - (KMAX - k)] = ok ? (int32_t)key_idx(sink.a[j]) : -1;
+    knn_idx[j - (KMAX - k)] = ok ? (int32_t)pos_of[key_idx(sink.a[j])] : -1;
     if (knn_d2) knn_d2[j - (KMAX - k)] = ok ? key_d2(sink.a[j]) : 0.f;
   }
 }
@@ -44,8 +44,7 @@
     float d_unseen;
     const bool cert = wave_search<S>(g, q.x, q.y, q.z, active, r, __int_as_float(0x7f800000), max_rounds, sink, &my->s, d_unseen);
     if (!active || (threadIdx.x & 63) >= QPW) continue;
-    const uint32_t i = __float_as_uint(q.w);
-    if (cert || LIST) store_knn(sink, knn_idx + (size_t)i * k, knn_d2 ? knn_d2 + (size_t)i * k : nullptr);
+    if (cert || LIST) store_knn(sink, knn_idx + (size_t)t * k, knn_d2 ? knn_d2 + (size_t)t * k : nullptr, g.pos_of);
     else {
       const uint32_t fs = atomicAdd(fb_count, 1u);
       fb_list[fs] = make_uint2(t, __float_as_uint(r));
diff --git a/fast-lio-sam-qn_amd/qn_amd/engine.py b/fast-lio-sam-qn_amd/qn_amd/engine.py
--- a/fast-lio-sam-qn_amd/qn_amd/engine.py
+++ b/fast-lio-sam-qn_amd/qn_amd/engine.py
@@ -268,6 +268,12 @@
         out = np.zeros((self._n[which], 3, 3))
         self.ctx.check(self._l.qn_gicp_get_covariances(self.ctx.h, C.c_int(which), _p(out)))
         return out
+
+    def source_normals(self):
+        n = self._n[0]
+        nrm = np.zeros((n, 3)); nrm_s = np.zeros((n, 3)); pos = np.zeros(n, dtype=np.uint32); sidx = np.zeros(n, dtype=np.uint32)
+        self.ctx.check(self._l.qn_debug_get_source_normals(self.ctx.h, _p(nrm), _p(nrm_s), _p(pos), _p(sidx)))
+        return nrm, nrm_s, pos, sidx
 
     def knn(self, which, k):
         idx = np.zeros((self._n[which], k), dtype=np.int32); d2 = np.zeros((self._n[which], k), dtype=np.float32)
diff --git a/include/qn_engine.h b/include/qn_engine.h
--- a/include/qn_engine.h
+++ b/include/qn_engine.h
@@ -305,6 +305,8 @@
 int  qn_debug_selftest(qn_ctx*, uint32_t n_waves, uint32_t seed, uint32_t* mismatches);
 int  qn_debug_get(qn_ctx*, const char* key, double* value);
 int  qn_debug_get_grid(qn_ctx*, int which, double out[8]);
+int  qn_debug_get_source_normals(qn_ctx*, double* nrm , double* nrm_sorted , uint32_t* pos_of ,
+                                 uint32_t* sorted_idx );
 int  qn_debug_get_partials(qn_ctx*, double* out, uint32_t* rows_per_buffer, double* state);
 int  qn_debug_get_list_probe(qn_ctx*, unsigned long long* out );
 int  qn_debug_get_persist_clk(qn_ctx*, unsigned long long* out );
```

Result: no change. 4410 (-0.6%).
